# emmyoh/zebra

Measured on AMD Instinct MI355X. Metric: queries/sec, higher is better.
Workload: dtype f32

## Files before the change

### include/zebra_hip.h

```cpp
#ifndef ZEBRA_HIP_H
#define ZEBRA_HIP_H

#include <stddef.h>
#include <stdint.h>

#ifdef __cplusplus
extern "C" {
#endif

#if defined(__GNUC__)
#define ZH_API __attribute__((visibility("default")))
#else
#define ZH_API
#endif

typedef struct zh_index zh_index;

typedef enum zh_status {
    ZH_OK = 0,
    ZH_EINVAL = -1,
    ZH_ENOMEM = -2,
    ZH_EHIP = -3,
    ZH_ESTATE = -4,
    ZH_ELIMIT = -5,
// ... 169 lines not shown
ZH_API int zh_distance_batch(int metric, int cosine_mode, const float *a, const float *q, size_t n, size_t dim,
                      uint64_t *out_keys, int device);
ZH_API int zh_distance_pair(int metric, int cosine_mode, const float *a, const float *b, size_t dim, uint64_t *out_key,
                     int device);

ZH_API int zh_merge_topk_device(int device, uint32_t n_shards, size_t b, size_t k, const uint64_t *d_ids,
                         const uint64_t *d_keys, const uint32_t *d_counts, uint64_t *d_out_ids,
                         uint64_t *d_out_keys, uint32_t *d_out_counts, void *stream);

ZH_API size_t zh_packed_result_words(size_t b, size_t k);
ZH_API int zh_merge_topk_packed_device(int device, uint32_t n_shards, size_t b, size_t k, const uint64_t *d_packed,
                                uint64_t *d_out_ids, uint64_t *d_out_keys, uint32_t *d_out_counts, void *stream);

typedef struct zh_shard_group zh_shard_group;
#define ZH_UNIQUE_ID_BYTES 128
ZH_API int zh_shard_unique_id(uint8_t out_id[ZH_UNIQUE_ID_BYTES]);
ZH_API int zh_shard_group_create(zh_index *shard, const uint8_t id[ZH_UNIQUE_ID_BYTES], uint32_t n_ranks, uint32_t rank,
                                 zh_shard_group **out);
ZH_API void zh_shard_group_destroy(zh_shard_group *grp);
ZH_API uint32_t zh_shard_group_ranks(const zh_shard_group *grp);
ZH_API uint32_t zh_shard_group_rank(const zh_shard_group *grp);
ZH_API int zh_shard_search_batch_device(zh_shard_group *grp, const float *d_q, size_t b, size_t k, int metric, int cosine_mode,
                                        uint64_t *d_out_ids, uint64_t *d_out_keys, uint32_t *d_out_counts);
ZH_API int zh_shard_search_batch(zh_shard_group *grp, const float *q, size_t b, size_t k, int metric, int cosine_mode,
                                 uint64_t *out_ids, uint64_t *out_keys, uint32_t *out_counts);
typedef struct zh_shard_ctx zh_shard_ctx;
ZH_API int zh_shard_ctx_create(zh_shard_group *grp, zh_shard_ctx **out);
ZH_API void zh_shard_ctx_destroy(zh_shard_ctx *ctx);
ZH_API int zh_shard_search_begin(zh_shard_ctx *ctx, const float *d_q, size_t b, size_t k, int metric, int cosine_mode);
ZH_API int zh_shard_search_finish(zh_shard_ctx *ctx, uint64_t *d_out_ids, uint64_t *d_out_keys, uint32_t *d_out_counts);
ZH_API int zh_shard_search_wait(zh_shard_ctx *ctx);
ZH_API int zh_shard_search_begin_window(zh_shard_ctx *ctx, const float *const *d_q, size_t n_batches, size_t b, size_t k,
                                        int metric, int cosine_mode);
ZH_API int zh_shard_search_finish_window(zh_shard_ctx *ctx, uint64_t *const *d_out_ids, uint64_t *const *d_out_keys,
                                         uint32_t *const *d_out_counts);
ZH_API void *zh_shard_ctx_stream(const zh_shard_ctx *ctx);
ZH_API const uint64_t *zh_shard_ctx_local_result(const zh_shard_ctx *ctx);
ZH_API size_t zh_shard_exchange_words(size_t b, size_t k);
ZH_API uint64_t zh_shard_status_word(int status, uint32_t visits_per_query);
ZH_API int zh_shard_verdict(const uint64_t *status_words, uint32_t n_ranks, uint32_t rank, uint32_t *out_first_failed_rank,
                            uint32_t *out_max_visits_per_query, int *out_all_elimit);

ZH_API int zh_synth_queries_device(int device, float *d_out, uint64_t seed_rows, uint64_t seed_q, uint64_t n_rows,
                            uint64_t b0, size_t b, uint32_t dim, int kind, void *stream);

typedef struct zh_ref_forest zh_ref_forest;
ZH_API int zh_ref_forest_decode(uint32_t dim, size_t n_trees, const uint8_t *const *values, const size_t *lens,
                                size_t n_vectors, const uint8_t *uuids, zh_ref_forest **out, uint64_t *out_unknown_ids);
ZH_API int zh_ref_forest_view(const zh_ref_forest *forest, zh_forest_view *out);
ZH_API void zh_ref_forest_free(zh_ref_forest *forest);
ZH_API int zh_ref_tree_encode(const zh_forest_view *forest, uint32_t dim, uint32_t tree, const uint8_t *uuids,
                              uint64_t n_rows, uint8_t *out, size_t cap, size_t *out_len);

typedef struct zh_ref_header {
    uint8_t uuid[16];
    uint64_t max_node_size;
    uint64_t num_trees;
    int32_t metric;
    int32_t power;
    uint64_t model_off, model_len;
} zh_ref_header;
ZH_API int zh_ref_header_decode(const uint8_t *bytes, size_t len, int metric, size_t model_len, zh_ref_header *out);
ZH_API int zh_ref_header_encode(const zh_ref_header *header, const uint8_t *model_bytes, uint8_t *out, size_t cap, size_t *out_len);

typedef struct zh_debug_pair {
    uint32_t row;
    uint32_t query;
    uint32_t lo, hi;
    float raw_s, raw_a2;
    uint32_t flags;
    uint32_t visit;
} zh_debug_pair;
typedef struct zh_debug_scan_info {
    uint32_t approx_scan;
    uint32_t queries, top_k;
    int32_t metric, cosine_mode;
    uint32_t raw_kept;
    uint32_t overflow;
    float bound_const;
    float row_rho, rho_norm;
    uint64_t pairs, visits;
} zh_debug_scan_info;
ZH_API int zh_debug_keep_raw(zh_index *idx, int on);
ZH_API int zh_debug_scan_pairs(zh_index *idx, zh_search_ctx *ctx, zh_debug_scan_info *info, zh_debug_pair *out, size_t cap, float *qmeta);

ZH_API int zh_set_profiling(zh_index *idx, int level);
ZH_API int zh_stats(zh_index *idx, zh_stats_t *out);
ZH_API int zh_stats_reset(zh_index *idx);
ZH_API int zh_set_dense_levels(zh_index *idx, int levels);
ZH_API int zh_set_sweep_mode(zh_index *idx, int mode);
ZH_API int zh_set_hash_mode(zh_index *idx, int mode);

ZH_API const char *zh_last_error(void);
ZH_API const char *zh_version(void);
ZH_API int zh_trim_device_memory(void);

#ifdef __cplusplus
}
#endif
#endif
```

### zebra_amd/_ffi.py

```python
import ctypes as C
import os

_HERE = os.path.dirname(os.path.abspath(__file__))
LIB_PATH = os.path.join(_HERE, "lib", "libzebra_hip.so")

ZH_OK = 0
ZH_EINVAL, ZH_ENOMEM, ZH_EHIP, ZH_ESTATE, ZH_ELIMIT, ZH_EUNSUPPORTED, ZH_EPEER = -1, -2, -3, -4, -5, -6, -7
COSINE, L2SQ, L2 = 0, 1, 2
CHEBYSHEV, CANBERRA, BRAY_CURTIS, MANHATTAN, L3, L4, HAMMING, MINKOWSKI, PNORM = 3, 4, 5, 6, 7, 8, 9, 10, 11
COSINE_PARITY, COSINE_CORRECTED = 0, 1
MAX_TOPK = 1024


class ZhError(RuntimeError):
    def __init__(self, code, msg):
        super().__init__(f"zebra_hip error {code}: {msg}")
        self.code = code


class Options(C.Structure):
    _fields_ = [("dim", C.c_uint32), ("max_node_size", C.c_uint32), ("num_trees", C.c_uint32),
                ("seed", C.c_uint64), ("device", C.c_int32), ("id_base", C.c_uint64),
                ("reserve_rows", C.c_uint64)]

# ... 58 lines not shown


class CompactInfo(C.Structure):
    _fields_ = [("rows_before", C.c_uint64), ("rows_after", C.c_uint64), ("rows_moved", C.c_uint64), ("bytes_moved", C.c_uint64),
                ("scratch_bytes", C.c_uint64), ("capacity_rows", C.c_uint64), ("copy_bytes_released", C.c_uint64), ("ms", C.c_double)]

    def as_dict(self):
        return {k: getattr(self, k) for k, _ in self._fields_}


COMPACT_BOUNCE_BYTES = 256 << 20

_vp, _u64, _u32, _sz, _i = C.c_void_p, C.c_uint64, C.c_uint32, C.c_size_t, C.c_int
SYMBOLS = [
    ("zh_options_default", None, [_vp]),
    ("zh_index_create", _i, [_vp, _vp]),
    ("zh_index_destroy", None, [_vp]),
    ("zh_index_clear", _i, [_vp]),
    ("zh_index_add", _i, [_vp, _vp, _sz, _vp]),
    ("zh_index_append", _i, [_vp, _vp, _sz, _vp]),
    ("zh_index_append_device", _i, [_vp, _vp, _sz]),
    ("zh_index_append_synthetic", _i, [_vp, _sz, _u64, _u64, _i]),
    ("zh_index_build", _i, [_vp]),
    ("zh_index_remove", _i, [_vp, _vp, _sz, _vp, _vp]),
    ("zh_index_deduplicate", _i, [_vp, _vp, _sz, _vp]),
    ("zh_index_compact", _i, [_vp, _vp, _sz, _vp]),
    ("zh_index_set_forest", _i, [_vp, _vp]),
    ("zh_index_forest_sizes", _i, [_vp, _vp]),
    ("zh_index_get_forest", _i, [_vp] * 8),
    ("zh_index_count", _u64, [_vp]),
    ("zh_index_num_trees", _u32, [_vp]),
    ("zh_index_stored_rows", _u64, [_vp]),
    ("zh_index_dim", _u32, [_vp]),
    ("zh_index_device", C.c_int32, [_vp]),
    ("zh_index_id_base", _u64, [_vp]),
    ("zh_index_rows_device", _vp, [_vp]),
    ("zh_index_sweep_stream", _vp, [_vp]),
    ("zh_index_read_rows", _i, [_vp, _u64, _sz, _vp]),
    ("zh_hash_signs", _i, [_vp, _vp, _sz, _vp, _vp]),
    ("zh_search_batch", _i, [_vp, _vp, _sz, _sz, _i, _i, _vp, _vp, _vp]),
    ("zh_search_batch_device", _i, [_vp, _vp, _sz, _sz, _i, _i, _vp, _vp, _vp, _vp]),
    ("zh_search_exact_batch", _i, [_vp, _vp, _sz, _sz, _i, _i, _vp, _vp, _vp]),
    ("zh_search_exact_batch_device", _i, [_vp, _vp, _sz, _sz, _i, _i, _vp, _vp, _vp, _vp]),
    ("zh_search_exact_info", _i, [_vp, _vp]),
    ("zh_search_ctx_create", _i, [_vp, _vp]),
    ("zh_search_ctx_destroy", None, [_vp]),
    ("zh_search_begin", _i, [_vp, _vp, _sz, _sz, _i, _i, _vp]),
    ("zh_search_finish", _i, [_vp, _vp, _vp, _vp, _vp]),
    ("zh_search_wait", _i, [_vp]),
    ("zh_search_begin_window", _i, [_vp, _vp, _sz, _sz, _sz, _i, _i, _vp]),
    ("zh_search_finish_window", _i, [_vp, _vp, _vp, _vp, _vp]),
    ("zh_distance_batch", _i, [_i, _i, _vp, _vp, _sz, _sz, _vp, _i]),
    ("zh_distance_pair", _i, [_i, _i, _vp, _vp, _sz, _vp, _i]),
    ("zh_merge_topk_device", _i, [_i, _u32, _sz, _sz, _vp, _vp, _vp, _vp, _vp, _vp, _vp]),
    ("zh_packed_result_words", _sz, [_sz, _sz]),
    ("zh_merge_topk_packed_device", _i, [_i, _u32, _sz, _sz, _vp, _vp, _vp, _vp, _vp]),
    ("zh_shard_unique_id", _i, [_vp]),
    ("zh_shard_group_create", _i, [_vp, _vp, _u32, _u32, _vp]),
    ("zh_shard_group_destroy", None, [_vp]),
    ("zh_shard_group_ranks", _u32, [_vp]),
    ("zh_shard_group_rank", _u32, [_vp]),
    ("zh_shard_search_batch_device", _i, [_vp, _vp, _sz, _sz, _i, _i, _vp, _vp, _vp]),
    ("zh_shard_search_batch", _i, [_vp, _vp, _sz, _sz, _i, _i, _vp, _vp, _vp]),
    ("zh_shard_ctx_create", _i, [_vp, _vp]),
    ("zh_shard_ctx_destroy", None, [_vp]),
    ("zh_shard_search_begin", _i, [_vp, _vp, _sz, _sz, _i, _i]),
    ("zh_shard_search_finish", _i, [_vp, _vp, _vp, _vp]),
    ("zh_shard_search_wait", _i, [_vp]),
    ("zh_shard_search_begin_window", _i, [_vp, _vp, _sz, _sz, _sz, _i, _i]),
    ("zh_shard_search_finish_window", _i, [_vp, _vp, _vp, _vp]),
    ("zh_shard_ctx_stream", _vp, [_vp]),
    ("zh_shard_ctx_local_result", _vp, [_vp]),
    ("zh_shard_exchange_words", _sz, [_sz, _sz]),
    ("zh_shard_status_word", _u64, [_i, _u32]),
    ("zh_shard_verdict", _i, [_vp, _u32, _u32, _vp, _vp, _vp]),
    ("zh_synth_queries_device", _i, [_i, _vp, _u64, _u64, _u64, _u64, _sz, _u32, _i, _vp]),
    ("zh_ref_forest_decode", _i, [_u32, _sz, _vp, _vp, _sz, _vp, _vp, _vp]),
    ("zh_ref_forest_view", _i, [_vp, _vp]),
    ("zh_ref_forest_free", None, [_vp]),
    ("zh_ref_tree_encode", _i, [_vp, _u32, _u32, _vp, _u64, _vp, _sz, _vp]),
    ("zh_ref_header_decode", _i, [_vp, _sz, _i, _sz, _vp]),
    ("zh_ref_header_encode", _i, [_vp, _vp, _vp, _sz, _vp]),
    ("zh_debug_keep_raw", _i, [_vp, _i]),
    ("zh_debug_scan_pairs", _i, [_vp, _vp, _vp, _vp, _sz, _vp]),
    ("zh_set_profiling", _i, [_vp, _i]),
    ("zh_stats", _i, [_vp, _vp]),
    ("zh_stats_reset", _i, [_vp]),
    ("zh_set_dense_levels", _i, [_vp, _i]),
    ("zh_set_sweep_mode", _i, [_vp, _i]),
    ("zh_set_hash_mode", _i, [_vp, _i]),
    ("zh_last_error", C.c_char_p, []),
    ("zh_version", C.c_char_p, []),
    ("zh_trim_device_memory", _i, []),
]

_lib = None


def lib():
    global _lib
    if _lib is None:
        if not os.path.exists(LIB_PATH):
            raise ImportError(f"{LIB_PATH} is missing: build it with `python -c 'import __graft_entry__ as g; "
                              f"g.build()'` or `make -C zebra_amd/csrc` (there is no CPU fallback)")
        L = C.CDLL(LIB_PATH)
        for name, res, args in SYMBOLS:
            fn = getattr(L, name)
            fn.restype = res
            fn.argtypes = args
        _lib = L
    return _lib


def check(rc):
    if rc != ZH_OK:
        raise ZhError(rc, lib().zh_last_error().decode("utf-8", "replace"))
```

### zebra_amd/csrc/zh_api.hip

```cpp
#include <algorithm>
#include <atomic>
#include <chrono>
#include <condition_variable>
#include <cmath>
#include <deque>
#include <cstdarg>
#include <cstdio>
#include <cstring>
#include <mutex>
#include <shared_mutex>
#include <new>
#include <string>
#include <thread>
#include <vector>

#include "zh_internal.h"

static thread_local std::string g_err;

static int fail(int code, const char *fmt, ...) {
    char buf[512];
    va_list ap;
    va_start(ap, fmt);
    vsnprintf(buf, sizeof buf, fmt, ap);
// ... 12 lines not shown
int zh_set_error(int code, const char *fmt, ...) {
    char buf[512];
    va_list ap;
    va_start(ap, fmt);
    vsnprintf(buf, sizeof buf, fmt, ap);
    va_end(ap);
    g_err = buf;
    return code;
}

extern "C" const char *zh_last_error(void) { return g_err.c_str(); }
extern "C" const char *zh_version(void) { return "zebra-hip 0.1 (gfx950)"; }

struct DevBuf {
    void *p = nullptr;
    size_t cap = 0;
    bool defer = false;
    std::vector<void *> old;
    size_t old_bytes = 0;
    int ensure(size_t bytes, bool keep = false, hipStream_t s = nullptr) {
        if (bytes <= cap) return ZH_OK;
        if (defer) bytes += bytes / 8;
        if (defer && old_bytes + cap > (size_t(2) << 30)) {
            for (void *o : old) hipFree(o);
            old.clear();
            old_bytes = 0;
        }
        size_t ncap = std::max(bytes, cap + cap / 2);
        ncap = (ncap + 255) & ~size_t(255);
        void *np = nullptr;
        hipError_t e = hipMalloc(&np, ncap);
        if (e != hipSuccess) {
            ncap = (bytes + 255) & ~size_t(255);
            e = hipMalloc(&np, ncap);
        }
        if (e != hipSuccess) return fail(ZH_ENOMEM, "hipMalloc(%zu bytes): %s", ncap, hipGetErrorString(e));
        if (keep && p && cap) {
            e = hipMemcpyAsync(np, p, cap, hipMemcpyDeviceToDevice, s);
            if (e == hipSuccess) e = hipStreamSynchronize(s);
            if (e != hipSuccess) { hipFree(np); return fail(ZH_EHIP, "grow copy: %s", hipGetErrorString(e)); }
        }
        if (p) { if (defer) { old.push_back(p); old_bytes += cap; } else hipFree(p); }
        p = np;
        cap = ncap;
        return ZH_OK;
    }
    void release() {
        if (p) hipFree(p);
        for (void *o : old) hipFree(o);
        old.clear();
        old_bytes = 0;
        p = nullptr;
        cap = 0;
    }
    template <typename T>
    T *as() const { return reinterpret_cast<T *>(p); }
};

struct zh_search_ctx {
    zh_index *ix = nullptr;
    DevBuf wQQ, wBits, wCounts, wInline, wRowBase, wCandBase, wVisitBase, wTotals, wVisits, wKeys, wCandKeys, wCandIds,
        wLeafCount, wLeafFill, wGroupBase, wGroupRowBase, wGroups, wGroupRowOff, wWaveGroup, wVisitBits, wNodeVisit, wScore, wJunkBits, wZeros, wQnorm, wQpad, wFixList, wLogPool, wLogHead, wLogCtl,
        wPfRows, wPfCounts, wPfKeys, wPfIds, wPfAmb, wPfCtl, wUnc, wQh, wQmeta, wApList, wApCount, wApEx, wApExKeys, wApCtl, wRaw;
    ZhApprox dbg_ap{};
    bool dbg_valid = false, dbg_raw = false;
    size_t log_chunks = 0;
    ZhTotals *h_totals = nullptr;
    hipEvent_t ev[6] = {};
    hipEvent_t ev_totals = nullptr, ev_emit = nullptr, ev_sw0 = nullptr, ev_sw1 = nullptr;
    bool ev_ok = false;
    int state = 0;
    bool trivial = false;
    const float *dQ = nullptr;
    size_t B = 0, k = 0;
    size_t nwin = 1, bwin = 0;
    DevBuf wQwin, wOutWin;
    int metric = 0, mode = 0;
    uint32_t P_dense = 0, wpq = 0;
    hipStream_t s = nullptr;
    ZhTotals tot{};
    bool scan = false;
    bool approx_f32rows = false;
    bool approx_fused = false;
    bool approx_bytes = false;
    bool approx = false, approx_mfma = false, approx_leaf = false;
    uint32_t *h_ap = nullptr;
    bool score_hash = false;
    uint32_t score_Bp = 0;
    bool lazy_fix = false;
    bool prefilter = false, prefilter_off_once = false, stream_ordered = false;
    uint32_t pf_cap = 0;
    uint32_t *h_pf = nullptr;
    std::vector<const float *> sv_q;
    std::vector<uint64_t *> sv_ids, sv_keys;
    std::vector<uint32_t *> sv_counts;
    hipStream_t sv_heavy = nullptr;
    std::vector<DevBuf *> all_bufs() {
        return {&wQQ, &wBits, &wCounts, &wInline, &wRowBase, &wCandBase, &wVisitBase, &wTotals, &wVisits, &wKeys,
                &wCandKeys, &wCandIds, &wLeafCount, &wLeafFill, &wGroupBase, &wGroupRowBase, &wGroups, &wGroupRowOff, &wWaveGroup, &wVisitBits, &wNodeVisit, &wScore, &wJunkBits, &wZeros, &wQnorm, &wQpad, &wFixList,
                &wLogPool, &wLogHead, &wLogCtl, &wQwin, &wOutWin, &wPfRows, &wPfCounts, &wPfKeys, &wPfIds, &wPfAmb, &wPfCtl, &wUnc,
                &wQh, &wQmeta, &wApList, &wApCount, &wApEx, &wApExKeys, &wApCtl, &wRaw};
    }
    void release_all() {
        for (DevBuf *b : all_bufs()) b->release();
        if (ev_ok) { for (auto &e : ev) hipEventDestroy(e); hipEventDestroy(ev_totals); hipEventDestroy(ev_emit); hipEventDestroy(ev_sw0); hipEventDestroy(ev_sw1); ev_ok = false; }
        if (h_totals) { hipHostFree(h_totals); h_totals = nullptr; }
        if (h_pf) { hipHostFree(h_pf); h_pf = nullptr; }
        if (h_ap) { hipHostFree(h_ap); h_ap = nullptr; }
    }
};

struct zh_index {
    zh_options opt{};
    int device = 0;
    hipStream_t stream = nullptr;
    hipStream_t sweep_stream = nullptr;
    std::shared_mutex mu;

    DevBuf X;
    uint64_t n_rows = 0;

    DevBuf node_plane, node_left, node_right, node_pack, roots, planes, consts, leaf_ids;
    uint32_t n_nodes = 0, n_planes = 0, n_trees = 0;
    uint64_t n_leaf_ids = 0;
    std::vector<int32_t> h_plane, h_left, h_right;
    std::vector<uint32_t> h_roots;
    std::vector<uint32_t> planes_below_level;
    std::vector<uint32_t> h_leaf_ids;
    std::vector<uint8_t> h_dead;
    uint64_t n_dead = 0;
    std::vector<uint32_t> h_live;
    uint64_t h_live_rows = ~0ull;
    uint64_t h_live_dead = ~0ull;
    uint64_t h_live_gen = ~0ull;
    uint64_t rows_gen = 1, dead_gen = 1;
    uint32_t max_leaf_len = 0;
    DevBuf blk_recs, blk_upper, blk_roots;
    uint32_t n_blocks = 0, n_upper = 0;
    bool blocks_valid = false;
    bool blocks_inner = false;
    size_t blk_recs_b = 0;
    std::mutex blk_mu;
    DevBuf row_leaf;
    bool row_leaf_valid = false, row_leaf_failed = false;
    std::atomic<uint32_t> batches_since_change{0};
    DevBuf row_half, row_meta, row_rho_dev;
    std::atomic<bool> row_half_failed{false};
    DevBuf row_half128;
    std::atomic<uint64_t> h128_rows{0}, h128_gen{0};
    int h128_ex = 0;
    float h128_rho = 0.f;
    std::atomic<bool> h128_failed{false};
    bool h128_bytes = false, h128_not_bytes = false;
    std::atomic<uint64_t> scale_rows{0}, scale_gen{0};
    float row_rho = 0.f;
    DevBuf scan_perm, row_leaf_p;
    bool row_order_off = false;
    uint32_t order_keys = 0;
    double order_worth = 0;
    uint64_t perm_rows = 0, row_leaf_gen = 0, row_leaf_p_gen = 0, perm_gen = 0, row_leaf_p_perm = 0;
    uint64_t row_leaf_rows = 0;

    zh_search_ctx dctx;
    DevBuf wQ, wOutIds, wOutKeys, wOutCounts;
    DevBuf ex_live, ex_bits, ex_QQ, ex_keys, ex_visits, ex_cbase, ex_ckeys, ex_cids, ex_run_ids, ex_run_keys, ex_run_counts, ex_Q, ex_ids, ex_kout, ex_counts,
        ex_Qh, ex_qmeta, ex_tau, ex_cnt, ex_lid, ex_llo, ex_lhi, ex_scr, ex_over;
    uint64_t ex_live_rows = ~0ull, ex_live_gen = ~0ull, ex_n_live = 0;
    zh_exact_info ex_info{};

    bool broken = false;
    bool rows_torn = false;
    int dense_levels = -1;
    bool debug_keep_raw = false;
    std::atomic<int> sweep_mode{0};
    std::atomic<uint32_t> approx_strikes{0};
    std::atomic<bool> mfma_f32_off{false};
    std::atomic<bool> fused_off{false};
    int hash_mode = 0;
    DevBuf plane_samples;
    bool samples_valid = false;
    DevBuf row_hn2, row_norm;
    uint64_t norm_rows = 0, norm_gen = 0;
    DevBuf plane_hab;
    uint32_t hab_planes = 0;
    uint64_t hab_rows = 0, hab_gen = 0;
    DevBuf leaf_meta;
    bool leaf_meta_valid = false;
    uint64_t meta_rows = 0, meta_gen = 0;
    std::atomic<uint32_t> prefilter_strikes{0};
    bool scan_unsafe = false;
    double visits_per_pair = 0;
    int profiling = 0;
    std::mutex stats_mu;
    zh_stats_t stats{};
    struct CombineReq {
        const float *q; size_t b, k; int metric, mode;
        uint64_t *ids, *keys; uint32_t *counts;
        int rc = 0; std::string err;
        std::mutex m; std::condition_variable cv; bool done = false, lead = false;
    };
    struct Lane {
        zh_search_ctx ctx;
        bool init = false, busy = false;
        hipStream_t s = nullptr;
        zh_search_ctx ctx2;
        bool init2 = false;
        hipStream_t s2 = nullptr;
        zh_search_ctx ctx3;
        bool init3 = false;
        hipStream_t s3 = nullptr;
        zh_search_ctx ctx4;
        bool init4 = false;
        hipStream_t s4 = nullptr;
        hipEvent_t ev_d2h[4] = {nullptr, nullptr, nullptr, nullptr};
        DevBuf wQ, wOutIds, wOutKeys, wOutCounts;
        void *h_stage = nullptr;
        size_t h_stage_cap = 0;
    };
    std::mutex cmu;
    std::deque<CombineReq *> cpend;
    bool cleader = false;
    size_t clast = 0;
    Lane lanes[1];
};

static const char *const k_torn_msg = "an earlier zh_index_compact failed after rows had begun to move: the stored rows are inconsistent; "
                                      "zh_index_clear the index and store them again";
static int set_device(const zh_index *ix) {
    hipError_t e = hipSetDevice(ix->device);
    if (e != hipSuccess) return fail(ZH_EHIP, "hipSetDevice(%d): %s", ix->device, hipGetErrorString(e));
    return ZH_OK;
}

static ZhForestDev forest_dev(const zh_index *ix) {
    ZhForestDev f;
    f.node_plane = ix->node_plane.as<int32_t>();
    f.node_left = ix->node_left.as<int32_t>();
    f.node_right = ix->node_right.as<int32_t>();
    f.node_pack = ix->node_pack.as<int4>();
    f.roots = ix->roots.as<uint32_t>();
    f.planes = ix->planes.as<float>();
    f.consts = ix->consts.as<float>();
    f.leaf_ids = ix->leaf_ids.as<uint32_t>();
    f.n_nodes = ix->n_nodes;
    f.n_planes = ix->n_planes;
    f.n_trees = ix->n_trees;
    f.group = zh_group_size(ix->opt.dim);
    return f;
}

static int ctx_init(zh_search_ctx *c, zh_index *ix) {
    c->ix = ix;
    for (DevBuf *b : c->all_bufs()) b->defer = true;
    hipError_t e = hipHostMalloc((void **)&c->h_totals, sizeof(ZhTotals), hipHostMallocDefault);
    if (e != hipSuccess) return fail(ZH_ENOMEM, "hipHostMalloc: %s", hipGetErrorString(e));
    e = hipHostMalloc((void **)&c->h_pf, 4 * sizeof(uint32_t), hipHostMallocDefault);
// ... 1836 lines not shown
                                   c->wCandBase.as<uint64_t>(), c->wVisitBase.as<uint64_t>(), c->wVisits.as<ZhVisit>(),
                                   c->wLeafCount.as<uint32_t>(), c->wLeafFill.as<uint32_t>(), c->wGroupBase.as<uint32_t>(),
                                   c->wGroupRowBase.as<uint64_t>(), c->wGroups.as<ZhGroup>(), c->wGroupRowOff.as<uint64_t>(), s));
        const uint64_t pairs = (uint64_t)B * T;
        const uint64_t want = tot.visits / (ZH_LOG_CHUNK - 1) + std::min<uint64_t>(pairs, tot.visits / (ZH_INLINE_VISITS + 1)) + 16;
        static const bool fixed = getenv("ZH_WALK_LOG_FIXED") != nullptr;
        if (!fixed && want > c->log_chunks) {
            const size_t chunks = (size_t)(want + want / 2);
            if (c->wLogPool.ensure(chunks * ZH_LOG_CHUNK * sizeof(uint2)) == ZH_OK) c->log_chunks = chunks;
        }
    }
    c->scan = choose_scan(ix, tot, c->metric, B, k);
    if (c->scan && (!ix->row_leaf_valid || ix->row_leaf_rows != ix->n_rows)) {
        std::lock_guard<std::mutex> lk(ix->blk_mu);
        if ((!ix->row_leaf_valid || ix->row_leaf_rows != ix->n_rows) && !ix->row_leaf_failed && (rc = build_row_leaf(ix))) return rc;
        if (!ix->row_leaf_valid || ix->row_leaf_rows != ix->n_rows) c->scan = false;
    }
    if (c->scan) {
        const size_t nn = std::max<uint32_t>(ix->n_nodes, 1);
        if ((rc = c->wVisitBits.ensure((nn + 31) / 32 * 4))) return rc;
        if ((rc = c->wNodeVisit.ensure(nn * sizeof(uint4)))) return rc;
        HIPCHK(zh_launch_node_visits(c->wLeafCount.as<uint32_t>(), c->wGroupBase.as<uint32_t>(), c->wGroups.as<ZhGroup>(), ix->n_nodes,
                                     c->wVisitBits.as<uint32_t>(), c->wNodeVisit.as<uint4>(), s));
    }
    if (!c->scan)
        HIPCHK(zh_launch_wave_groups(c->wGroups.as<ZhGroup>(), c->wGroupRowOff.as<uint64_t>(), tot.groups, c->wWaveGroup.as<uint32_t>(), s));
    c->approx = c->scan && use_approx(ix, tot, B, k, c->metric);
    c->approx_leaf = false; c->approx_bytes = false;
    if (!c->scan && use_approx_leaf(ix, tot, B, k, c->metric)) {
        bool ok = false;
        const char *be = getenv("ZH_S128H_BYTES"), *ke = getenv("ZH_S128H_KERNEL"), *de = getenv("ZH_S128H_DMA");
        const bool want_bytes = !(be && be[0] == '0') && !(ke && ke[0] == 'r') && !(de && de[0] == '1');
        std::lock_guard<std::mutex> lk(ix->blk_mu);
        if ((rc = ensure_row_half128(ix, &ok, want_bytes))) return rc;
        c->approx = c->approx_leaf = ok;
        c->approx_bytes = ok && ix->h128_bytes;
    }
    ZhApprox ap{};
    bool mfma = c->approx && !c->approx_leaf && mfma_wanted(ix) && B < (1u << 23) - 1;
    const uint2 *scan_row_leaf = ix->row_leaf.as<uint2>();
    if (mfma) {
        std::lock_guard<std::mutex> lk(ix->blk_mu);
        if ((rc = ensure_row_half(ix, &mfma))) return rc;
        if (mfma && ix->perm_rows) {
            if ((rc = ensure_row_leaf_p(ix))) return rc;
            if (!ix->perm_rows) {
                ix->row_order_off = true;
                ix->scale_gen = 0;
                if ((rc = ensure_row_half(ix, &mfma))) return rc;
            } else
                scan_row_leaf = ix->row_leaf_p.as<uint2>();
        }
    }
    c->approx_mfma = mfma;
    c->approx_f32rows = mfma && ix->row_half.p == nullptr;
    if (c->approx) {
        const char *cap_e = getenv("ZH_APX_CAPS");
        unsigned e_capq = 0, e_excap = 0, e_exrows = 0;
        if (cap_e) sscanf(cap_e, "%u,%u,%u", &e_capq, &e_excap, &e_exrows);
        const uint32_t capq = e_capq ? std::min(e_capq, 8192u) : (ix->approx_strikes.load() ? 8192u : 4096u);
        const uint32_t ex_cap = e_excap ? e_excap : (uint32_t)std::min<uint64_t>(std::max<uint64_t>(4096, tot.visits / 4 + 1024), 1u << 24);
        const uint32_t ex_rows = e_exrows ? e_exrows : (uint32_t)std::min<uint64_t>(std::max<uint64_t>(1u << 20, tot.rows / 16), 1u << 26);
        if ((rc = c->wQh.ensure(B * d * 2)) || (rc = c->wQmeta.ensure(B * sizeof(float4))) || (rc = c->wApList.ensure((size_t)B * capq * 12)) ||
            (rc = c->wApCount.ensure(B * 8 + std::max<uint64_t>(tot.visits, 1) * 4)) || (rc = c->wApEx.ensure((size_t)ex_cap * 8)) || (rc = c->wApExKeys.ensure((size_t)ex_rows * 20)) ||
            (rc = c->wApCtl.ensure(ZH_APX_CTL_WORDS * 4)))
            return rc;
        ap.Qh = c->wQh.p; ap.qmeta = c->wQmeta.as<float4>(); ap.iv = c->wKeys.as<uint64_t>();
        ap.list_lo = c->wApList.as<uint32_t>(); ap.list_hi = ap.list_lo + (size_t)B * capq; ap.list_id = ap.list_hi + (size_t)B * capq;
        ap.qcount = c->wApCount.as<uint32_t>(); ap.capq = capq; ap.qtau = ap.qcount + B; ap.tauv = ap.qtau + B;
        ap.ex_visits = c->wApEx.as<uint2>(); ap.ex_cap = ex_cap;
        ap.ex_keys = c->wApExKeys.as<uint64_t>(); ap.ex_ckeys = ap.ex_keys + ex_rows; ap.ex_cids = reinterpret_cast<uint32_t *>(ap.ex_ckeys + ex_rows);
        ap.ex_rows_cap = ex_rows; ap.ctl = c->wApCtl.as<uint32_t>();
        ap.n_queries = (uint32_t)B; ap.iv_cap = tot.rows;
        ap.mfma = mfma ? 1u : 0u; ap.row_half = mfma ? ix->row_half.p : nullptr; ap.row_meta = mfma ? ix->row_meta.as<float2>() : nullptr;
        ap.row_rho = mfma ? ix->row_rho : 0.f;
        if (c->approx_leaf) { ap.mfma = 2u; ap.row_rho = ap.rho_norm = c->approx_bytes ? 0.f : ix->h128_rho; }
        const char *pte = getenv("ZH_S128H_PRETEST");
        ap.nx_max = c->approx_leaf && c->approx_bytes && !(pte && pte[0] == '0') ? 2885.1f : 0.f;
        HIPCHK(hipMemsetAsync(c->wApCount.p, 0, B * 4, s));
        HIPCHK(hipMemsetAsync(ap.qtau, 0xFF, B * 4, s));
        HIPCHK(hipMemsetAsync(c->wApCtl.p, 0, ZH_APX_CTL_WORDS * 4, s));
        HIPCHK(zh_launch_qhalf(c->dQ, (uint32_t)B, d, c->wQh.p, c->wQmeta.as<float4>(), c->approx_leaf ? 2 : (mfma ? 1 : 0), s));
    }
    HIPCHK(hipEventRecord(c->ev[2], s));
    hipStream_t hs = heavy ? heavy : s;
    if (hs != s) { HIPCHK(hipEventRecord(c->ev_emit, s)); HIPCHK(hipStreamWaitEvent(hs, c->ev_emit, 0)); }
    HIPCHK(hipEventRecord(c->ev_sw0, hs));
    c->approx_fused = false;
    if (c->approx_leaf && k <= 64 && !ix->debug_keep_raw) {
        const char *fe = getenv("ZH_S128H_FUSED"), *ke = getenv("ZH_S128H_KERNEL"), *de = getenv("ZH_S128H_DMA");
        const bool lean = !(ke && ke[0] == 'r') && !(de && de[0] == '1');
        c->approx_fused = lean && (fe ? fe[0] == '1' : (!ix->fused_off && tot.rows >= 1024 * std::max<uint64_t>(tot.visits, 1)));
    }
    const int kinda = c->metric != ZH_COSINE ? 0 : (c->mode == ZH_COSINE_PARITY ? 2 : 1);
    if (c->approx_leaf)
        HIPCHK(zh_launch_sweep128h(ix->row_half128.p, c->wQh.p, ldexpf(1.f, ix->h128_ex - 14), c->wGroups.as<ZhGroup>(), c->wGroupRowOff.as<uint64_t>(),
                                   tot.groups, c->wWaveGroup.as<uint32_t>(), f.leaf_ids, tot.group_rows, c->wKeys.as<uint64_t>(), hs,
                                   c->approx_fused ? &ap : nullptr, kinda, (uint32_t)k, zh_approx_bound(c->metric, d, 2), c->approx_bytes));
    else if (c->approx)
        HIPCHK(zh_launch_scan_approx(ix->X.as<float>(), d, ix->n_rows, ap, mfma ? scan_row_leaf : ix->row_leaf.as<uint2>(), T, c->wVisitBits.as<uint32_t>(),
                                     c->wNodeVisit.as<uint4>(), c->wGroups.as<ZhGroup>(), f.group, c->metric, c->mode, hs));
    else if (c->scan)
        HIPCHK(zh_launch_scan_sweep(ix->X.as<float>(), d, ix->n_rows, c->dQ, c->wQQ.as<float>(), ix->row_leaf.as<uint2>(), T,
                                    c->wVisitBits.as<uint32_t>(), c->wNodeVisit.as<uint4>(), c->wGroups.as<ZhGroup>(), f.group,
                                    c->metric, c->mode, c->wKeys.as<uint64_t>(), nullptr, hs));
    else
        HIPCHK(zh_launch_sweep(ix->X.as<float>(), d, c->dQ, c->wQQ.as<float>(), c->wGroups.as<ZhGroup>(),
                               c->wGroupRowOff.as<uint64_t>(), tot.groups, c->wWaveGroup.as<uint32_t>(), f.leaf_ids,
                               tot.group_rows, c->metric, c->mode, c->wKeys.as<uint64_t>(), hs));
    HIPCHK(hipEventRecord(c->ev_sw1, hs));
    if (hs != s) HIPCHK(hipStreamWaitEvent(s, c->ev_sw1, 0));
    HIPCHK(hipEventRecord(c->ev[3], s));
    const uint32_t *run_if = nullptr;
    c->dbg_valid = c->approx;
    c->dbg_raw = false;
    if (c->approx) {
        c->dbg_ap = ap;
        if (ix->debug_keep_raw && tot.rows) {
            if ((rc = c->wRaw.ensure(tot.rows * 8))) return rc;
            HIPCHK(hipMemcpyAsync(c->wRaw.p, c->wKeys.p, tot.rows * 8, hipMemcpyDeviceToDevice, s));
            c->dbg_raw = true;
        }
        if (c->approx_fused) HIPCHK(zh_launch_exact_register(c->wVisits.as<ZhVisit>(), tot.visits, (uint32_t)k, ap, s));
        else HIPCHK(zh_launch_select_interval(c->wVisits.as<ZhVisit>(), tot.visits, (uint32_t)k, f.leaf_ids, ap, c->metric, c->mode, d, s));
        HIPCHK(hipEventRecord(c->ev[4], s));
        HIPCHK(zh_launch_final_interval(c->wVisits.as<ZhVisit>(), ix->X.as<float>(), d, c->dQ, c->wQQ.as<float>(), (uint32_t)B, (uint32_t)k,
                                        f.leaf_ids, c->metric, c->mode, ix->opt.id_base, ap, dOutIds, dOutKeys, dOutCounts, ix->max_leaf_len, s));
        HIPCHK(hipMemcpyAsync(c->h_ap, c->wApCtl.p, ZH_APX_CTL_WORDS * 4, hipMemcpyDeviceToHost, s));
        run_if = ap.ctl + 1;
        if (c->approx_leaf)
            HIPCHK(zh_launch_sweep(ix->X.as<float>(), d, c->dQ, c->wQQ.as<float>(), c->wGroups.as<ZhGroup>(), c->wGroupRowOff.as<uint64_t>(), tot.groups,
                                   c->wWaveGroup.as<uint32_t>(), f.leaf_ids, tot.group_rows, c->metric, c->mode, c->wKeys.as<uint64_t>(), s, run_if));
        else
            HIPCHK(zh_launch_scan_sweep(ix->X.as<float>(), d, ix->n_rows, c->dQ, c->wQQ.as<float>(), ix->row_leaf.as<uint2>(), T,
                                        c->wVisitBits.as<uint32_t>(), c->wNodeVisit.as<uint4>(), c->wGroups.as<ZhGroup>(), f.group,
                                        c->metric, c->mode, c->wKeys.as<uint64_t>(), run_if, s));
    }
    HIPCHK(zh_launch_select(c->wVisits.as<ZhVisit>(), tot.visits, f.leaf_ids, c->wKeys.as<uint64_t>(),
                            c->wCandKeys.as<uint64_t>(), c->wCandIds.as<uint32_t>(), ix->max_leaf_len, run_if, s));
    if (!c->approx) HIPCHK(hipEventRecord(c->ev[4], s));
    HIPCHK(zh_launch_final(c->wCandBase.as<uint64_t>(), (uint32_t)B, T, (uint32_t)k, c->wCandKeys.as<uint64_t>(),
                           c->wCandIds.as<uint32_t>(), ix->opt.id_base, dOutIds, dOutKeys, dOutCounts, run_if, s));
    for (size_t j = 0; j < nwin && nwin > 1; j++) {
        HIPCHK(hipMemcpyAsync(outIds[j], dOutIds + j * bwin * k, bwin * k * 8, hipMemcpyDeviceToDevice, s));
        HIPCHK(hipMemcpyAsync(outKeys[j], dOutKeys + j * bwin * k, bwin * k * 8, hipMemcpyDeviceToDevice, s));
        HIPCHK(hipMemcpyAsync(outCounts[j], dOutCounts + j * bwin, bwin * 4, hipMemcpyDeviceToDevice, s));
    }
    HIPCHK(hipEventRecord(c->ev[5], s));
    c->state = 2;
    return ZH_OK;
}

int ctx_wait(zh_search_ctx *c) {
    zh_index *ix = c->ix;
    if (c->state == 1) return fail(ZH_ESTATE, "zh_search_wait: the batch was begun but not finished");
    if (c->state != 2) return ZH_OK;
    c->state = 0;
    HIPCHK(hipEventSynchronize(c->ev[5]));
    if (c->trivial) return ZH_OK;
    const bool pf = c->prefilter;
    const uint32_t pf_amb = pf ? c->h_pf[0] : 0, pf_flags = pf ? c->h_pf[1] : 0, pf_exact = pf ? c->h_pf[2] : 0;
    if (pf_flags) {
        {
            std::lock_guard<std::mutex> lk(ix->stats_mu);
            ix->stats.prefilter_fallbacks_accum++;
            ix->stats.prefilter_last_overflow = pf_flags;
        }
        ix->prefilter_strikes.fetch_add(1);
        const std::vector<const float *> q = c->sv_q;
        const std::vector<uint64_t *> ids = c->sv_ids, keys = c->sv_keys;
        const std::vector<uint32_t *> counts = c->sv_counts;
        c->prefilter_off_once = true;
        int rc = ctx_begin(c, q.data(), c->nwin, c->bwin, c->k, c->metric, c->mode, c->s);
        if (!rc) rc = ctx_finish(c, ids.data(), keys.data(), counts.data(), c->sv_heavy);
        c->prefilter_off_once = false;
        if (rc) return rc;
        return ctx_wait(c);
    }
    if (pf) ix->prefilter_strikes = 0;
    const ZhTotals tot = c->tot;
    uint64_t uniq = 0;
    if (ix->profiling >= 2 && tot.visits && !pf) {
        std::vector<ZhVisit> hv(tot.visits);
        HIPCHK(hipMemcpy(hv.data(), c->wVisits.p, tot.visits * sizeof(ZhVisit), hipMemcpyDeviceToHost));
// ... 110 lines not shown

extern "C" int zh_search_ctx_create(zh_index *ix, zh_search_ctx **out) {
    if (!ix || !out) return fail(ZH_EINVAL, "zh_search_ctx_create: null argument");
    int rc = set_device(ix);
    if (rc) return rc;
    zh_search_ctx *c = new (std::nothrow) zh_search_ctx();
    if (!c) return fail(ZH_ENOMEM, "out of host memory");
    if ((rc = ctx_init(c, ix))) { c->release_all(); delete c; return rc; }
    *out = c;
    return ZH_OK;
}
extern "C" void zh_search_ctx_destroy(zh_search_ctx *c) {
    if (!c) return;
    hipSetDevice(c->ix->device);
    if (c->state == 2) hipEventSynchronize(c->ev[5]);
    else if (c->state == 1 && c->s) hipStreamSynchronize(c->s);
    c->release_all();
    delete c;
}
extern "C" int zh_search_begin(zh_search_ctx *c, const float *d_q, size_t b, size_t k, int metric, int mode, void *stream) {
    if (!c || (b && !d_q)) return fail(ZH_EINVAL, "zh_search_begin: null argument");
    if (k > ZH_MAX_TOPK) return fail(ZH_ELIMIT, "top_k %zu > ZH_MAX_TOPK (%u)", k, ZH_MAX_TOPK);
    int rc = check_metric(metric, mode);
    if (rc) return rc;
    if ((rc = set_device(c->ix))) return rc;
    return ctx_begin(c, &d_q, 1, b, k, metric, mode, stream ? (hipStream_t)stream : c->ix->stream);
}
extern "C" int zh_search_begin_window(zh_search_ctx *c, const float *const *d_q, size_t n_batches, size_t b, size_t k, int metric,
                                      int mode, void *stream) {
    if (!c || !d_q || n_batches == 0 || n_batches > ZH_MAX_WINDOW) return fail(ZH_EINVAL, "zh_search_begin_window: bad argument (1..%u batches)", ZH_MAX_WINDOW);
    for (size_t j = 0; j < n_batches; j++)
        if (b && !d_q[j]) return fail(ZH_EINVAL, "zh_search_begin_window: null query pointer");
    if (k > ZH_MAX_TOPK) return fail(ZH_ELIMIT, "top_k %zu > ZH_MAX_TOPK (%u)", k, ZH_MAX_TOPK);
    int rc = check_metric(metric, mode);
    if (rc) return rc;
    if ((rc = set_device(c->ix))) return rc;
    return ctx_begin(c, d_q, n_batches, b, k, metric, mode, stream ? (hipStream_t)stream : c->ix->stream);
}
extern "C" int zh_search_finish(zh_search_ctx *c, uint64_t *d_out_ids, uint64_t *d_out_keys, uint32_t *d_out_counts,
                                void *sweep_stream) {
    if (!c) return fail(ZH_EINVAL, "zh_search_finish: null context");
    if (c->B && (!d_out_counts || (c->k && (!d_out_ids || !d_out_keys)))) return fail(ZH_EINVAL, "zh_search_finish: null output");
    if (c->nwin != 1) return fail(ZH_ESTATE, "zh_search_finish: the context holds a window; use zh_search_finish_window");
    int rc = set_device(c->ix);
    if (rc) return rc;
    return ctx_finish(c, &d_out_ids, &d_out_keys, &d_out_counts, (hipStream_t)sweep_stream);
}
extern "C" int zh_search_finish_window(zh_search_ctx *c, uint64_t *const *d_out_ids, uint64_t *const *d_out_keys,
                                       uint32_t *const *d_out_counts, void *sweep_stream) {
    if (!c || !d_out_ids || !d_out_keys || !d_out_counts) return fail(ZH_EINVAL, "zh_search_finish_window: null argument");
    for (size_t j = 0; j < c->nwin && c->bwin; j++)
        if (!d_out_counts[j] || (c->k && (!d_out_ids[j] || !d_out_keys[j]))) return fail(ZH_EINVAL, "zh_search_finish_window: null output");
    int rc = set_device(c->ix);
    if (rc) return rc;
    return ctx_finish(c, d_out_ids, d_out_keys, d_out_counts, (hipStream_t)sweep_stream);
}
double zh_index_visits_per_pair(zh_index *ix) {
    std::lock_guard<std::mutex> lk(ix->stats_mu);
    return ix->visits_per_pair;
}
void zh_search_ctx_stream_ordered(zh_search_ctx *c) {
    if (c) c->stream_ordered = true;
}
void zh_search_ctx_abandon(zh_search_ctx *c) {
    if (c && c->state == 1) c->state = 0;
}
extern "C" int zh_search_wait(zh_search_ctx *c) {
    if (!c) return fail(ZH_EINVAL, "zh_search_wait: null context");
    int rc = set_device(c->ix);
    if (rc) return rc;
    return ctx_wait(c);
}

extern "C" int zh_trim_device_memory(void) {
    return ZH_OK;
}

extern "C" int zh_debug_keep_raw(zh_index *ix, int on) {
    if (!ix) return fail(ZH_EINVAL, "zh_debug_keep_raw: null index");
    std::unique_lock<std::shared_mutex> lk(ix->mu);
    ix->debug_keep_raw = on != 0;
    return ZH_OK;
}
extern "C" int zh_debug_scan_pairs(zh_index *ix, zh_search_ctx *ctx, zh_debug_scan_info *info, zh_debug_pair *out, size_t cap, float *qmeta) {
    if (!ix || !info || (cap && !out)) return fail(ZH_EINVAL, "zh_debug_scan_pairs: null argument");
    std::unique_lock<std::shared_mutex> lk(ix->mu, std::defer_lock);
    if (!ctx) lk.lock();
    zh_search_ctx *c = ctx ? ctx : &ix->dctx;
    if (c->ix != ix) return fail(ZH_EINVAL, "zh_debug_scan_pairs: the context belongs to another index");
    if (c->state != 0) return fail(ZH_ESTATE, "zh_debug_scan_pairs: the context has a batch in flight");
    int rc = set_device(ix);
    if (rc) return rc;
    memset(info, 0, sizeof(*info));
    if (!c->dbg_valid) return ZH_OK;
    if (c->approx_leaf && c->approx_fused)
        return fail(ZH_ESTATE, "zh_debug_scan_pairs: the batch's sweep was fused (no per-pair results exist); call zh_debug_keep_raw(idx, 1) first");
    const ZhTotals tot = c->tot;
    const ZhApprox &ap = c->dbg_ap;
    info->approx_scan = c->approx_leaf ? 3 : (c->approx_mfma ? 2 : 1);
    info->queries = (uint32_t)c->B; info->top_k = (uint32_t)c->k; info->metric = c->metric; info->cosine_mode = c->mode;
    info->raw_kept = c->dbg_raw ? 1 : 0; info->overflow = c->h_ap[1];
    info->bound_const = zh_approx_bound(c->metric, ix->opt.dim, (int)ap.mfma);
    info->row_rho = ap.row_rho; info->rho_norm = ap.rho_norm;
    info->pairs = tot.rows; info->visits = tot.visits;
    HIPCHK(hipDeviceSynchronize());
    if (qmeta) HIPCHK(hipMemcpy(qmeta, ap.qmeta, c->B * sizeof(float4), hipMemcpyDeviceToHost));
    if (!cap) return ZH_OK;
    if (cap < tot.rows) return fail(ZH_ELIMIT, "zh_debug_scan_pairs: %llu pairs, room for %zu", (unsigned long long)tot.rows, cap);
    std::vector<ZhVisit> hv(tot.visits);
    std::vector<uint64_t> iv(tot.rows), raw(c->dbg_raw ? tot.rows : 0);
    std::vector<uint32_t> lids(ix->n_leaf_ids);
    if (tot.visits) HIPCHK(hipMemcpy(hv.data(), c->wVisits.p, tot.visits * sizeof(ZhVisit), hipMemcpyDeviceToHost));
    if (tot.rows) HIPCHK(hipMemcpy(iv.data(), c->wKeys.p, tot.rows * 8, hipMemcpyDeviceToHost));
    if (c->dbg_raw && tot.rows) HIPCHK(hipMemcpy(raw.data(), c->wRaw.p, tot.rows * 8, hipMemcpyDeviceToHost));
    if (ix->n_leaf_ids) HIPCHK(hipMemcpy(lids.data(), ix->leaf_ids.p, ix->n_leaf_ids * 4, hipMemcpyDeviceToHost));
    for (size_t i = 0; i < tot.rows; i++) { out[i].row = out[i].query = 0xFFFFFFFFu; out[i].flags = 0; out[i].visit = 0xFFFFFFFFu; }
    for (size_t v = 0; v < hv.size(); v++) {
        const ZhVisit &z = hv[v];
        if (z.row_off + z.len > tot.rows || (uint64_t)z.leaf_off + z.len > ix->n_leaf_ids) return fail(ZH_ESTATE, "zh_debug_scan_pairs: visit %zu out of range", v);
        const uint32_t fl = (z.take ? 1u : 0u) | ((z.take && z.take < z.len && z.take < c->k) ? 2u : 0u);
        for (uint32_t i = 0; i < z.len; i++) {
            zh_debug_pair &o = out[z.row_off + i];
            o.row = lids[(size_t)z.leaf_off + i]; o.query = z.b; o.visit = (uint32_t)v; o.flags = fl;
            const uint64_t w = iv[z.row_off + i];
            o.lo = (uint32_t)w; o.hi = (uint32_t)(w >> 32);
            o.raw_s = o.raw_a2 = 0.f;
            if (c->dbg_raw) { const uint64_t r = raw[z.row_off + i]; uint32_t a = (uint32_t)r, b2 = (uint32_t)(r >> 32); memcpy(&o.raw_s, &a, 4); memcpy(&o.raw_a2, &b2, 4); }
        }
    }
    return ZH_OK;
}

static size_t host_window_queries(const zh_index *ix, bool wander) {
    const char *e = getenv("ZH_HOST_WINDOW");
    const size_t forced = e ? (size_t)atoll(e) : (size_t)0;
    if (forced) return forced;
    const uint32_t d = ix->opt.dim;
    if (wander) {
        const size_t w = ((size_t)1 << 28) / std::max<uint64_t>(ix->n_rows, 1) / 64 * 64;
        return std::min<size_t>(std::max<size_t>(w, 64), 1024);
    }
    return d >= 512 ? 2048 : (d >= 256 ? 1024 : 4096);
}
static size_t host_windows_wanted(zh_index *ix, size_t B, size_t k, bool *wander) {
    const bool off = getenv("ZH_NO_HOST_WINDOWS") != nullptr;
    if (off || ix->n_trees == 0 || ix->n_rows == 0) return 0;
    double vpp;
    {
        std::lock_guard<std::mutex> lk(ix->stats_mu);
        vpp = ix->visits_per_pair;
    }
    if (!(vpp > 0)) {
        if ((size_t)ix->opt.max_node_size >= 2 * k + 2) return 0;
        vpp = 1000.0;
    }
    const size_t wq = host_window_queries(ix, vpp > 4.0);
    if (B < 2 * wq && B < wq + wq / 2) return 0;
    *wander = vpp > 4.0;
    return wq;
}
#ifndef ZH_HOST_AHEAD_WANDER
#define ZH_HOST_AHEAD_WANDER 2
#endif
static int search_host_windows(zh_index *ix, zh_index::Lane &ln, size_t wq, int ahead, const float *q, size_t B, size_t k, int metric, int mode, uint64_t *out_ids,
                               uint64_t *out_keys, uint32_t *out_counts) {
    const uint32_t d = ix->opt.dim;
    int rc;
    auto init_ctx = [&](zh_search_ctx *c, hipStream_t *st, bool *flag) -> int {
        if (*flag) return ZH_OK;
        int r = ctx_init(c, ix);
        if (r) { c->release_all(); return r; }
        int lo = 0, hi = 0;
        hipDeviceGetStreamPriorityRange(&lo, &hi);
        hipError_t e = hipStreamCreateWithPriority(st, hipStreamNonBlocking, hi);
        for (auto &ev : ln.ev_d2h)
            if (e == hipSuccess && !ev) e = hipEventCreateWithFlags(&ev, hipEventDisableTiming);
        if (e != hipSuccess) {
            c->release_all();
            if (*st) { hipStreamDestroy(*st); *st = nullptr; }
            return fail(ZH_EHIP, "host windows: %s", hipGetErrorString(e));
        }
        *flag = true;
        return ZH_OK;
    };
    if ((rc = init_ctx(&ln.ctx2, &ln.s2, &ln.init2))) return rc;
    if (ahead >= 1 && init_ctx(&ln.ctx3, &ln.s3, &ln.init3) != ZH_OK) ahead = 0;
    if (ahead >= 2 && init_ctx(&ln.ctx4, &ln.s4, &ln.init4) != ZH_OK) ahead = 1;
    const int NC = 2 + ahead;
    const size_t A = (size_t)ahead;
    const size_t nw = (B + wq - 1) / wq, per = (B + nw - 1) / nw;
    const size_t off_ids = B * d * 4, off_keys = off_ids + B * k * 8, off_counts = off_keys + B * k * 8, need = off_counts + B * 4;
    if (need > ln.h_stage_cap) {
        if (ln.h_stage) hipHostFree(ln.h_stage);
        ln.h_stage = nullptr; ln.h_stage_cap = 0;
        const size_t cap = need + need / 2;
        hipError_t e = hipHostMalloc(&ln.h_stage, cap, hipHostMallocDefault);
        if (e != hipSuccess) return fail(ZH_ENOMEM, "hipHostMalloc(%zu): %s", cap, hipGetErrorString(e));
        ln.h_stage_cap = cap;
    }
    uint8_t *hs = static_cast<uint8_t *>(ln.h_stage);
    float *dQ = ln.wQ.as<float>();
    uint64_t *dIds = ln.wOutIds.as<uint64_t>(), *dKeys = ln.wOutKeys.as<uint64_t>();
    uint32_t *dCounts = ln.wOutCounts.as<uint32_t>();
    uint64_t *hIds = reinterpret_cast<uint64_t *>(hs + off_ids), *hKeys = reinterpret_cast<uint64_t *>(hs + off_keys);
    uint32_t *hCounts = reinterpret_cast<uint32_t *>(hs + off_counts);
    zh_search_ctx *ctxs[4] = {&ln.ctx, &ln.ctx2, &ln.ctx3, &ln.ctx4};
    hipStream_t str[4] = {ln.s, ln.s2, ln.s3, ln.s4};
    auto win = [&](size_t w, size_t *b0, size_t *nb) { *b0 = w * per; *nb = std::min(per, B - *b0); };
// ... 601 lines not shown
```

### zebra_amd/csrc/zh_approx.hip

```cpp

#include <cstdlib>

#include "zh_internal.h"
#include "zh_device.h"

typedef _Float16 f16x8 __attribute__((ext_vector_type(8)));

#ifndef ZH_APX_G768
#define ZH_APX_G768 2
#endif
#ifndef ZH_APX_G128
#define ZH_APX_G128 8
#endif
uint32_t zh_approx_groups(uint32_t d) {
    switch (d) {
    case 128: return ZH_APX_G128;
    case 256: case 384: return 4;
    case 768: return ZH_APX_G768;
    case 512: case 1024: return 2;
    default: return 0;
    }
}
bool zh_approx_pays(uint32_t d) { return d >= 384; }

float zh_approx_bound(int metric, uint32_t d, int mfma) {
    const double u = 5.9604644775390625e-8, c0 = (d + 255) / 256 + 8.0, ops = mfma ? 33.0 * (d / 128) + 2.0 + (mfma == 2 ? 40.0 : 0.0) : 0.0;
    if (metric == ZH_COSINE) return (float)(1.01 * (2.0 * c0 + 80.0 + 2.0 * ops) * u);
    return (float)(1.01 * (c0 + 100.0 + ops) * u);
}

__device__ __forceinline__ _Float16 f16_no_subnormal(float v) {
    const _Float16 h = (_Float16)v;
    return fabsf((float)h) < 6.103515625e-05f ? (_Float16)0.f : h;
}

template <int G>
__global__ __launch_bounds__(64) void qhalf_kernel(const float *__restrict__ Q, uint32_t B, uint32_t d, _Float16 *__restrict__ Qh,
                                                    float4 *__restrict__ qmeta) {
    constexpr uint32_t LG = 64 / G;
    const uint32_t b = blockIdx.x, lane = threadIdx.x;
    const float *q = Q + (size_t)b * d;
    float m = 0.f, s2 = 0.f;
    bool bad = false;
    for (uint32_t e = lane; e < d; e += 64) {
        const float v = q[e];
        bad |= !(v - v == 0.f);
        m = fmaxf(m, fabsf(v));
        s2 = __builtin_fmaf(v, v, s2);
    }
    m = wave_butterfly<OpMax>(m);
    s2 = wave_sum_canonical(s2);
    bad = __ballot(bad) != 0;
    float sigma = 1.f, inv = 1.f;
    if (!bad && m > 0.f) {
        int ex = 0;
        (void)frexpf(m, &ex);
        if (ex < -90 || ex > 90) bad = true;
        else { sigma = ldexpf(1.f, 14 - ex); inv = ldexpf(1.f, ex - 14); }
    }
    float d2 = 0.f;
    for (uint32_t e = lane; e < d; e += 64) {
        const float v = bad ? 0.f : q[e];
        const _Float16 h = f16_no_subnormal(v * sigma);
        const float df = v - (float)h * inv;
        d2 = __builtin_fmaf(df, df, d2);
        const uint32_t j = e / (4 * LG), rem = e % (4 * LG), l = rem / 4, t = rem % 4, i = j / 2, wh = j % 2;
        Qh[(size_t)b * d + ((size_t)(i * LG + l)) * 8 + wh * 4 + t] = h;
    }
    d2 = wave_sum_canonical(d2);
    if (lane == 0) {
        float4 o;
        if (bad || !(s2 - s2 == 0.f)) o = make_float4(NAN, NAN, NAN, NAN);
        else o = make_float4(inv, s2, sqrtf(s2) * (1.0f + 1e-5f), sqrtf(d2) * 1.001f);
        qmeta[b] = o;
    }
}

hipError_t zh_launch_qhalf(const float *dQ, uint32_t B, uint32_t d, void *dQh, float4 *dQmeta, int layout, hipStream_t s) {
    if (!B) return hipSuccess;
    const uint32_t G = layout == 2 ? 64 : (layout == 1 ? 16 : zh_approx_groups(d));
    if (G == 64) hipLaunchKernelGGL(qhalf_kernel<64>, dim3(B), dim3(64), 0, s, dQ, B, d, (_Float16 *)dQh, dQmeta);
    else if (G == 16) hipLaunchKernelGGL(qhalf_kernel<16>, dim3(B), dim3(64), 0, s, dQ, B, d, (_Float16 *)dQh, dQmeta);
    else if (G == 8) hipLaunchKernelGGL(qhalf_kernel<8>, dim3(B), dim3(64), 0, s, dQ, B, d, (_Float16 *)dQh, dQmeta);
// ... 272 lines not shown
        const uint64_t row = row0 + i;
        const float *x = X + (size_t)(perm && row < perm_rows ? perm[row] : row) * d;
        float m = 0.f, a2 = 0.f;
        bool bad = false;
        for (uint32_t e = lane; e < d; e += 64) {
            const float v = x[e];
            bad |= !(v - v == 0.f);
            m = fmaxf(m, fabsf(v));
            a2 = __builtin_fmaf(v, v, a2);
        }
        m = wave_butterfly<OpMax>(m);
        a2 = wave_sum_canonical(a2);
        bad = __ballot(bad) != 0;
        bool usable = false;
        float sigma = 1.f, inv = __uint_as_float(0x7FC00000u);
        if (!bad) {
            int ex = 14;
            if (m > 0.f) (void)frexpf(m, &ex);
            if (ex >= -100 && ex <= 100) { usable = true; sigma = ldexpf(1.f, 14 - ex); inv = ldexpf(1.f, ex - 14); }
        }
        float s2 = 0.f, d2 = 0.f;
        _Float16 *tile = Xh + ((size_t)(row >> 4) * NS * 64 + (row & 15)) * 8;
        for (uint32_t e = lane; e < d; e += 64) {
            const float v = x[e] * sigma;
            const _Float16 hv = usable ? f16_no_subnormal(v) : (_Float16)0.f;
            const float df = v - (float)hv;
            s2 = __builtin_fmaf(v, v, s2);
            d2 = __builtin_fmaf(df, df, d2);
            const uint32_t st = e >> 5, w = e & 31, hh = (w & 15) >> 2, j = (w & 3) + ((w >> 4) << 2);
            if (Xh) tile[((size_t)st * 64 + hh * 16) * 8 + j] = hv;
        }
        s2 = wave_sum_canonical(s2);
        d2 = wave_sum_canonical(d2);
        if (usable && s2 > 0.f) rho_w = fmaxf(rho_w, sqrtf(d2) * 1.001f / (sqrtf(s2) * 0.9999f));
        if (lane == 0) rowMeta[row] = make_float2(a2, inv);
    }
    if (lane == 0 && rho_w > 0.f) atomicMax(rhoMax, __float_as_uint(rho_w));
}

hipError_t zh_launch_row_half(const float *dX, uint64_t row0, uint64_t n_rows, uint32_t d, void *dXh, float2 *dRowMeta, uint32_t *dRhoMax,
                              const uint32_t *dPerm, uint64_t perm_rows, hipStream_t s) {
    if (!n_rows) return hipSuccess;
    const uint64_t blocks = std::min<uint64_t>((n_rows + 3) / 4, 256 * 32);
    hipLaunchKernelGGL(row_half_kernel, dim3((uint32_t)blocks), dim3(256), 0, s, dX, row0, n_rows, d, (_Float16 *)dXh, dRowMeta, dRhoMax, dPerm, perm_rows);
    return hipGetLastError();
}

__global__ __launch_bounds__(256) void permute_row_leaf_kernel(const uint2 *__restrict__ rowLeaf, const uint32_t *__restrict__ perm, uint64_t perm_rows,
                                                               uint64_t n_entries, uint32_t T, uint2 *__restrict__ out) {
    for (uint64_t e = (uint64_t)blockIdx.x * blockDim.x + threadIdx.x; e < n_entries; e += (uint64_t)gridDim.x * blockDim.x) {
        const uint64_t p = e / T, t = e % T;
        out[e] = rowLeaf[(size_t)(p < perm_rows ? perm[p] : p) * T + t];
    }
}
hipError_t zh_launch_permute_row_leaf(const uint2 *dRowLeaf, const uint32_t *dPerm, uint64_t perm_rows, uint64_t n_rows, uint32_t T, uint2 *dOut, hipStream_t s) {
    const uint64_t n = n_rows * T;
    if (!n) return hipSuccess;
    hipLaunchKernelGGL(permute_row_leaf_kernel, dim3((uint32_t)std::min<uint64_t>((n + 255) / 256, 256 * 64)), dim3(256), 0, s, dRowLeaf, dPerm, perm_rows, n, T, dOut);
    return hipGetLastError();
}

#ifndef ZH_MFMA_CL
#define ZH_MFMA_CL 0
#endif
#ifdef ZH_SCAN_GUARD
#define ZH_GUARD(cond, bit) ((cond) ? true : (atomicOr(guard, (bit)), false))
#else
#define ZH_GUARD(cond, bit) true
#endif
#ifdef ZH_SCAN_PROF
__device__ unsigned long long zh_scan_prof_buf[16];
extern "C" __attribute__((visibility("default"))) int zh_debug_scan_prof(uint64_t *out, uint32_t words, int reset) {
    static const unsigned long long zero[16] = {};
    if (reset) return (int)hipMemcpyToSymbol(HIP_SYMBOL(zh_scan_prof_buf), zero, sizeof(zero));
    return (int)hipMemcpyFromSymbol(out, HIP_SYMBOL(zh_scan_prof_buf), (size_t)words * 8);
}
#define SP(...) __VA_ARGS__
#else
#define SP(...)
#endif
#ifndef ZH_MFMA_WAVES
#define ZH_MFMA_WAVES 3
#endif
template <int D, bool F32ROWS>
__global__ __launch_bounds__(256) __attribute__((amdgpu_waves_per_eu(D > 768 ? 2 : ZH_MFMA_WAVES, D > 768 ? 2 : ZH_MFMA_WAVES)))
void scan_mfma_kernel(const u32x4v *__restrict__ Xh, const float *__restrict__ Xf, const float2 *__restrict__ rowMeta,
                                                         const uint4 *__restrict__ Qh, const uint2 *__restrict__ rowLeaf, uint32_t T,
                                                         uint32_t RW, const uint32_t *__restrict__ visitBits,
                                                         const uint4 *__restrict__ nodeVisit, const ZhGroup *__restrict__ groups,
                                                         uint32_t GRP, uint64_t row_begin, uint64_t row_end, uint64_t *__restrict__ iv,
                                                         uint32_t *__restrict__ colStats ,
                                                         uint32_t nq, uint64_t iv_cap, uint32_t *__restrict__ guard) {
    constexpr int NS = D / 32;
    constexpr int NL = D / 64;
    constexpr int CL = ZH_MFMA_CL ? ZH_MFMA_CL : (NL % 4 == 0 ? 2 : 3);
    constexpr int NCH = NL / CL;
    static_assert(D % 128 == 0 && NL % CL == 0 && NCH % 2 == 0, "four accumulators; the chunk registers alternate with a static parity");
    __shared__ uint64_t pair_list[4][ZH_APX_CAP > CL * 256 ? ZH_APX_CAP : CL * 256];
    __shared__ uint64_t tile_list[4][ZH_APX_CAP];
    __shared__ uint32_t col_query[4][ZH_APX_CAP];
    __shared__ uint32_t tile_start[4][36];
    __shared__ f32x4v acc_lds[4][64];
    __shared__ float2 row_meta[4][16];
    const uint32_t lane = threadIdx.x & 63, c16 = lane & 15, h = lane >> 4;
    const uint32_t wid = (uint32_t)__builtin_amdgcn_readfirstlane((int)(threadIdx.x >> 6));
    const uint64_t wave = (uint64_t)blockIdx.x * (blockDim.x >> 6) + wid;
    const uint64_t r0 = row_begin + wave * RW;
    if (r0 >= row_end) return;
    SP(const uint64_t sp0 = clock64();)
    const uint32_t nr = (uint32_t)(row_end - r0 < RW ? row_end - r0 : RW);
    const uint32_t n_ent = nr * T;
    const uint2 *__restrict__ ent = rowLeaf + (size_t)r0 * T;
    uint32_t eGb[ZH_SCAN_NE], eWithin[ZH_SCAN_NE], eC[ZH_SCAN_NE], off[ZH_SCAN_NE], eB0[ZH_SCAN_NE];
    uint64_t eK0[ZH_SCAN_NE];
    const uint32_t P = scan_phase1(lane, n_ent, ent, visitBits, nodeVisit, eGb, eWithin, eC, off, eB0, eK0);
    if (P == 0) return;
    SP(const uint64_t sp1 = clock64();)
    uint64_t *list = pair_list[wid];
    const bool listed = P <= ZH_APX_CAP;
    auto pack = [](uint32_t rl, uint32_t b, uint64_t slot) { return slot | ((uint64_t)b << 36) | ((uint64_t)rl << 60); };
#pragma unroll
    for (int j = 0; j < ZH_SCAN_NE; j++) {
        const uint32_t e = lane + 64u * j, c = eC[j];
        if (c && listed && ZH_GUARD(off[j] + c <= (uint32_t)ZH_APX_CAP && e / T < 16u, 32u)) {
            const uint32_t rl = e / T, gb = eGb[j];
            list[off[j]] = pack(rl, eB0[j], eK0[j] + eWithin[j]);
            for (uint32_t sidx = 1; sidx < c; sidx++) {
                const ZhGroup *gp = groups + gb + sidx / GRP;
                list[off[j] + sidx] = pack(rl, gp->b[sidx % GRP], gp->key_off[sidx % GRP] + eWithin[j]);
            }
        }
    }
    SP(__builtin_amdgcn_s_waitcnt(0); const uint64_t sp2 = clock64();)
    f16x8 A[NS];
    if constexpr (!F32ROWS) {
        const u32x4v *tp = Xh + (size_t)(r0 >> 4) * (NS * 64) + lane;
#pragma unroll
        for (int st = 0; st < NS; st++) A[st] = __builtin_bit_cast(f16x8, __builtin_nontemporal_load(tp + 64 * st));
        if (lane < 16) row_meta[wid][lane] = rowMeta[r0 + (lane < nr ? lane : 0u)];
        __builtin_amdgcn_fence(__ATOMIC_RELEASE, "wavefront");
        __builtin_amdgcn_wave_barrier();
    } else {
        if (lane < 16) row_meta[wid][lane] = rowMeta[r0 + (lane < nr ? lane : 0u)];
        __builtin_amdgcn_fence(__ATOMIC_RELEASE, "wavefront");
        __builtin_amdgcn_wave_barrier();
        const float inv_c = row_meta[wid][c16].y;
        const bool usable_c = inv_c - inv_c == 0.f;
        const float sigma_c = usable_c ? 1.0f / inv_c : 0.f;
        f32x4v *xt = reinterpret_cast<f32x4v *>(tile_list[wid]);
        const f32x4v *X4 = reinterpret_cast<const f32x4v *>(Xf);
        const uint32_t g4 = lane >> 4, p16 = lane & 15;
        auto cvt8 = [&](const f32x4v lo, const f32x4v hi) {
            f16x8 o;
#pragma unroll
            for (int t = 0; t < 4; t++) {
                o[t] = usable_c ? f16_no_subnormal(lo[t] * sigma_c) : (_Float16)0.f;
                o[4 + t] = usable_c ? f16_no_subnormal(hi[t] * sigma_c) : (_Float16)0.f;
            }
            return o;
        };
        f32x4v Rr[4];
        auto issue_rows = [&](int kb) {
#pragma unroll
            for (int i = 0; i < 4; i++) {
                const uint32_t rr = 4u * i + g4;
                Rr[i] = __builtin_nontemporal_load(X4 + (size_t)(r0 + (rr < nr ? rr : nr - 1)) * (D / 4) + kb * 16 + p16);
            }
        };
        issue_rows(0);
#pragma unroll
        for (int kb = 0; kb < D / 64; kb++) {
#pragma unroll
            for (int i = 0; i < 4; i++) {
                const uint32_t rr = 4u * i + g4;
                xt[rr * 16 + (p16 ^ rr)] = Rr[i];
            }
            __builtin_amdgcn_fence(__ATOMIC_RELEASE, "wavefront");
            __builtin_amdgcn_wave_barrier();
            if (kb + 1 < D / 64) issue_rows(kb + 1);
#pragma unroll
            for (int s2 = 0; s2 < 2; s2++) {
                const f32x4v lo = xt[c16 * 16 + ((8u * s2 + h) ^ c16)], hi = xt[c16 * 16 + ((8u * s2 + 4u + h) ^ c16)];
                A[2 * kb + s2] = cvt8(lo, hi);
            }
            __builtin_amdgcn_fence(__ATOMIC_RELEASE, "wavefront");
            __builtin_amdgcn_wave_barrier();
        }
    }
    const float2 *rmeta = row_meta[wid];
    u32x4v *stg = reinterpret_cast<u32x4v *>(pair_list[wid]);
    const u32x4v *__restrict__ Qv = reinterpret_cast<const u32x4v *>(Qh);
    const uint32_t g8 = lane >> 3, pc = lane & 7;
    const uint32_t swA = (g8 >> 1) & 7u, swB = (4u + (g8 >> 1)) & 7u;
    const uint32_t rd0 = (c16 >> 3) * 64u + (c16 & 7u) * 8u + ((h ^ (c16 >> 1)) & 7u);
    const uint32_t rd1 = (c16 >> 3) * 64u + (c16 & 7u) * 8u + (((4u + h) ^ (c16 >> 1)) & 7u);
    auto issue = [&](uint32_t bA, uint32_t bB, int chunk, u32x4v *dst) {
        if (!ZH_GUARD(bA < nq && bB < nq, 1u)) { bA = 0; bB = 0; }
        const u32x4v *qa = Qv + (size_t)bA * (D / 8) + (size_t)(chunk * CL * 8) + (pc ^ swA);
        const u32x4v *qb = Qv + (size_t)bB * (D / 8) + (size_t)(chunk * CL * 8) + (pc ^ swB);
#pragma unroll
        for (int i = 0; i < CL; i++) { dst[2 * i] = qa[8 * i]; dst[2 * i + 1] = qb[8 * i]; }
    };
    auto to_lds = [&](const u32x4v *src) {
#pragma unroll
        for (int i = 0; i < 2 * CL; i++) stg[64 * i + lane] = src[i];
    };
    auto mfma_chunk = [&](int chunk, f32x4v *acc) {
#pragma unroll
        for (int i = 0; i < 2 * CL; i++) {
            const u32x4v v = stg[128 * (i / 2) + ((i & 1) ? rd1 : rd0)];
            const int st = chunk * 2 * CL + i;
            acc[st & 3] = __builtin_amdgcn_mfma_f32_16x16x32_f16(A[st], __builtin_bit_cast(f16x8, v), acc[st & 3], 0, 0, 0);
        }
    };
    auto emit = [&](const f32x4v *acc, uint32_t rl, uint64_t slot, bool valid) {
        const f32x4v t = (acc[0] + acc[1]) + (acc[2] + acc[3]);
        if (valid && (rl >> 2) == h) {
            const uint32_t i = rl & 3u;
            const float sv = i == 0 ? t[0] : (i == 1 ? t[1] : (i == 2 ? t[2] : t[3]));
            const float2 rm = rmeta[rl];
            if (ZH_GUARD(slot < iv_cap, 2u))
                __builtin_nontemporal_store(((uint64_t)__float_as_uint(rm.x) << 32) | __float_as_uint(sv * rm.y), iv + slot);
        }
    };
    if (listed) {
        uint32_t *tab = reinterpret_cast<uint32_t *>(tile_list[wid]);
        uint32_t *colq = col_query[wid], *tstart = tile_start[wid];
#pragma unroll
        for (int i = 0; i < 4; i++) reinterpret_cast<uint4 *>(tab)[lane + 64 * i] = make_uint4(0u, 0u, 0u, 0u);
        if (lane < 36) tstart[lane] = 0u;
        __builtin_amdgcn_fence(__ATOMIC_RELEASE, "wavefront");
        __builtin_amdgcn_wave_barrier();
        auto hash_of = [](uint32_t b) { return (b * 2654435761u) >> 22; };
        uint32_t nd = 0;
        for (uint32_t p0 = 0; p0 < P; p0 += 64) {
            const uint32_t pi = p0 + lane;
            const bool valid = pi < P;
            const uint32_t b = valid ? (uint32_t)(list[pi] >> 36) & 0xFFFFFFu : 0u, key = b + 1u;
            uint32_t hs = hash_of(b);
            bool leader = false, open = valid;
            while (__ballot(open)) {
                if (open) {
                    const uint32_t old = atomicCAS(&tab[hs], 0u, (key << 9) | 0x1FFu);
                    if (old == 0u) { leader = true; open = false; }
                    else if ((old >> 9) == key) open = false;
                    else hs = (hs + 1u) & 1023u;
                }
            }
            const unsigned long long lm = __ballot(leader);
            if (leader) {
                const uint32_t col = nd + (uint32_t)__builtin_popcountll(lm & ((1ull << lane) - 1ull));
                if (ZH_GUARD(col < (uint32_t)ZH_APX_CAP && hs < 1024u, 64u)) {
                    tab[hs] = (key << 9) | col;
                    colq[col] = b;
                }
            }
            nd += (uint32_t)__builtin_popcountll(lm);
        }
        __builtin_amdgcn_fence(__ATOMIC_RELEASE, "wavefront");
        __builtin_amdgcn_wave_barrier();
        for (uint32_t p0 = 0; p0 < P; p0 += 64) {
            const uint32_t pi = p0 + lane;
            if (pi < P) {
                const uint64_t rec = list[pi];
                const uint32_t b = (uint32_t)(rec >> 36) & 0xFFFFFFu, key = b + 1u;
                uint32_t hs = hash_of(b), w = tab[hs];
                for (uint32_t tries = 0; (w >> 9) != key && ZH_GUARD(tries < 1024u, 16u); tries++) { (void)tries; hs = (hs + 1u) & 1023u; w = tab[hs]; }
                const uint32_t col = w & 0x1FFu;
                if (!ZH_GUARD((w >> 9) == key && col < nd, 128u)) continue;
                const uint32_t pos = atomicAdd(&tstart[1 + (col >> 4)], 1u);
                list[pi] = (rec & ~(0xFFFFFFull << 36)) | ((uint64_t)(col | (pos << 9)) << 36);
            }
        }
        __builtin_amdgcn_fence(__ATOMIC_RELEASE, "wavefront");
        __builtin_amdgcn_wave_barrier();
        {
            uint32_t v = lane < 33 ? tstart[lane] : 0u;
#pragma unroll
            for (int o = 1; o < 64; o <<= 1) {
                const uint32_t u = __shfl_up(v, o);
                if (lane >= (uint32_t)o) v += u;
            }
            __builtin_amdgcn_wave_barrier();
            if (lane < 33) tstart[lane] = v;
        }
        __builtin_amdgcn_fence(__ATOMIC_RELEASE, "wavefront");
        __builtin_amdgcn_wave_barrier();
        uint64_t *tl = tile_list[wid];
        {
            uint64_t recs[ZH_APX_CAP / 64];
#pragma unroll
            for (int i = 0; i < ZH_APX_CAP / 64; i++) recs[i] = (uint32_t)(64 * i) + lane < P ? list[64 * i + lane] : ~0ull;
            __builtin_amdgcn_wave_barrier();
#pragma unroll
            for (int i = 0; i < ZH_APX_CAP / 64; i++)
                if ((uint32_t)(64 * i) + lane < P) {
                    const uint32_t cp = (uint32_t)(recs[i] >> 36) & 0xFFFFFFu, col = cp & 0x1FFu, pos = (cp >> 9) & 0x1FFu;
                    if (ZH_GUARD(tstart[col >> 4] + pos < (uint32_t)ZH_APX_CAP && col < nd, 4u | (col < nd ? 0u : 8u))) tl[tstart[col >> 4] + pos] = recs[i];
                }
        }
        __builtin_amdgcn_fence(__ATOMIC_RELEASE, "wavefront");
        __builtin_amdgcn_wave_barrier();
        const uint32_t nt = (nd + 15) / 16;
        SP(const uint64_t sp3 = clock64();)
        if (colStats && lane == 0 && (wave & 63u) == 0u) { atomicAdd(&colStats[0], nd); atomicAdd(&colStats[1], P); }
        auto col_b = [&](uint32_t t, uint32_t col) { const uint32_t ci = 16 * t + col; return colq[ci < nd ? ci : nd - 1]; };
        uint32_t bA = col_b(0, g8), bB = col_b(0, 8 + g8);
        u32x4v ra[2 * CL], rb[2 * CL];
        issue(bA, bB, 0, ra);
        SP(__builtin_amdgcn_s_waitcnt(0); const uint64_t sp4 = clock64();)
        f32x4v *al = acc_lds[wid];
        for (uint32_t t = 0; t < nt; t++) {
            f32x4v acc[4] = {{0.f, 0.f, 0.f, 0.f}, {0.f, 0.f, 0.f, 0.f}, {0.f, 0.f, 0.f, 0.f}, {0.f, 0.f, 0.f, 0.f}};
#pragma unroll
            for (int c = 0; c < NCH; c += 2) {
                issue(bA, bB, c + 1, rb);
                to_lds(ra);
                mfma_chunk(c, acc);
                if (c + 2 < NCH) issue(bA, bB, c + 2, ra);
                else {
                    bA = col_b(t + 1, g8); bB = col_b(t + 1, 8 + g8);
                    issue(bA, bB, 0, ra);
                }
                to_lds(rb);
                mfma_chunk(c + 1, acc);
            }
            al[c16 * 4 + h] = (acc[0] + acc[1]) + (acc[2] + acc[3]);
            __builtin_amdgcn_fence(__ATOMIC_RELEASE, "wavefront");
            __builtin_amdgcn_wave_barrier();
            const uint32_t pe = tstart[t + 1];
            for (uint32_t pi = tstart[t] + lane; pi < pe; pi += 64) {
                const uint64_t rec = tl[pi];
                const uint32_t rl = (uint32_t)(rec >> 60), col = (uint32_t)(rec >> 36) & 15u;
                const float sv = reinterpret_cast<const float *>(al)[col * 16 + rl];
                const float2 rm = rmeta[rl];
                if (ZH_GUARD((rec & 0xFFFFFFFFFull) < iv_cap, 2u))
                    __builtin_nontemporal_store(((uint64_t)__float_as_uint(rm.x) << 32) | __float_as_uint(sv * rm.y), iv + (rec & 0xFFFFFFFFFull));
            }
            __builtin_amdgcn_wave_barrier();
        }
        SP(if ((wave & 15u) == 0u && lane == 0) {
            __builtin_amdgcn_s_waitcnt(0);
            const uint64_t sp5 = clock64();
            atomicAdd(&zh_scan_prof_buf[0], 1ull); atomicAdd(&zh_scan_prof_buf[1], sp1 - sp0); atomicAdd(&zh_scan_prof_buf[2], sp2 - sp1);
            atomicAdd(&zh_scan_prof_buf[3], sp3 - sp2); atomicAdd(&zh_scan_prof_buf[4], sp4 - sp3); atomicAdd(&zh_scan_prof_buf[5], sp5 - sp4);
            atomicAdd(&zh_scan_prof_buf[6], (unsigned long long)nt); atomicAdd(&zh_scan_prof_buf[7], (unsigned long long)P);
            atomicAdd(&zh_scan_prof_buf[8], (unsigned long long)nd); atomicAdd(&zh_scan_prof_buf[9], sp5 - sp0);
        })
    } else {
#pragma unroll
        for (int j = 0; j < ZH_SCAN_NE; j++) {
            unsigned long long m = __ballot(eC[j] != 0);
            while (m) {
                const int ll = __builtin_ctzll(m);
                m &= m - 1;
                const uint32_t c = (uint32_t)__builtin_amdgcn_readlane((int)eC[j], ll);
                const uint32_t gb = (uint32_t)__builtin_amdgcn_readlane((int)eGb[j], ll);
                const uint32_t w = (uint32_t)__builtin_amdgcn_readlane((int)eWithin[j], ll);
                const uint32_t rl = ((uint32_t)ll + 64u * j) / T;
                for (uint32_t s0 = 0; s0 < c; s0 += 16) {
                    auto visit_b = [&](uint32_t col) { const uint32_t si = s0 + col < c ? s0 + col : c - 1; return groups[gb + si / GRP].b[si % GRP]; };
                    const uint32_t bA = visit_b(g8), bB = visit_b(8 + g8);
                    const uint32_t sidx = s0 + c16 < c ? s0 + c16 : c - 1;
                    const ZhGroup *gp = groups + gb + sidx / GRP;
                    f32x4v acc[4] = {{0.f, 0.f, 0.f, 0.f}, {0.f, 0.f, 0.f, 0.f}, {0.f, 0.f, 0.f, 0.f}, {0.f, 0.f, 0.f, 0.f}};
                    u32x4v rq[2 * CL];
#pragma unroll
                    for (int cc = 0; cc < NCH; cc++) {
                        issue(bA, bB, cc, rq);
                        to_lds(rq);
                        mfma_chunk(cc, acc);
                        __builtin_amdgcn_sched_barrier(0);
                    }
                    emit(acc, rl, gp->key_off[sidx % GRP] + w, s0 + c16 < c);
                }
            }
        }
    }
}

template <int D>
static hipError_t launch_scan_mfma_d(const float *dX, uint64_t n_rows, const ZhApprox &ap, const uint2 *dRowLeaf, uint32_t T,
                                     const uint32_t *dVisitBits, const uint4 *dNodeVisit, const ZhGroup *dGroups, uint32_t group, hipStream_t s) {
    const uint32_t RW = zh_scan_rows_per_wave(T);
    uint64_t rows_per_launch = zh_sweep_rows_per_launch(D);
    rows_per_launch = rows_per_launch / (4 * RW) * (4 * RW);
    for (uint64_t r = 0; r < n_rows; r += rows_per_launch) {
        const uint64_t r_end = r + rows_per_launch < n_rows ? r + rows_per_launch : n_rows;
        const uint64_t waves = (r_end - r + RW - 1) / RW, blocks = (waves + 3) / 4;
        if (blocks > 0x7FFFFFFFull) return hipErrorInvalidValue;
        if (ap.row_half)
            hipLaunchKernelGGL((scan_mfma_kernel<D, false>), dim3((uint32_t)blocks), dim3(256), 0, s, (const u32x4v *)ap.row_half, dX, ap.row_meta, (const uint4 *)ap.Qh, dRowLeaf, T, RW,
                               dVisitBits, dNodeVisit, dGroups, group, r, r_end, ap.iv, ap.ctl + 5, ap.n_queries, ap.iv_cap, ap.ctl + 7);
        else
            hipLaunchKernelGGL((scan_mfma_kernel<D, true>), dim3((uint32_t)blocks), dim3(256), 0, s, (const u32x4v *)nullptr, dX, ap.row_meta, (const uint4 *)ap.Qh, dRowLeaf, T, RW,
                               dVisitBits, dNodeVisit, dGroups, group, r, r_end, ap.iv, ap.ctl + 5, ap.n_queries, ap.iv_cap, ap.ctl + 7);
    }
    return hipGetLastError();
}

__global__ __launch_bounds__(256) void absmax_kernel(const float *__restrict__ X, uint64_t n, uint32_t *__restrict__ out) {
    float m = 0.f;
    for (uint64_t i = (uint64_t)blockIdx.x * blockDim.x + threadIdx.x; i < n; i += (uint64_t)gridDim.x * blockDim.x) {
        const float v = fabsf(X[i]);
        if (v - v == 0.f) m = fmaxf(m, v);
    }
    m = wave_butterfly<OpMax>(m);
    if ((threadIdx.x & 63) == 0 && m > 0.f) atomicMax(out, __float_as_uint(m));
}

__global__ __launch_bounds__(256) void row_half128_kernel(const float *__restrict__ X, uint64_t row0, uint64_t n_rows, float sigma,
                                                          _Float16 *__restrict__ Xh, uint32_t *__restrict__ rhoMax) {
    const uint32_t lane = threadIdx.x & 63;
    const uint64_t nw = (uint64_t)gridDim.x * 4;
    float rho_w = 0.f;
    for (uint64_t i = (uint64_t)blockIdx.x * 4 + (threadIdx.x >> 6); i < n_rows; i += nw) {
        const uint64_t row = row0 + i;
        const float2 x = reinterpret_cast<const float2 *>(X + (size_t)row * 128)[lane];
        const float v0 = x.x * sigma, v1 = x.y * sigma;
        bool bad = !(v0 - v0 == 0.f) || !(v1 - v1 == 0.f) || fabsf(v0) > 60000.f || fabsf(v1) > 60000.f;
        const _Float16 h0 = f16_no_subnormal(v0), h1 = f16_no_subnormal(v1);
        const float d0 = v0 - (float)h0, d1 = v1 - (float)h1;
        const float s2 = wave_sum_canonical(__builtin_fmaf(v0, v0, v1 * v1));
        const float d2 = wave_sum_canonical(__builtin_fmaf(d0, d0, d1 * d1));
        const float m = wave_butterfly<OpMax>(fmaxf(fabsf(x.x), fabsf(x.y)));
        bad = __ballot(bad) != 0 || !(s2 - s2 == 0.f) || (s2 == 0.f && m > 0.f);
        const float rho = s2 > 0.f ? sqrtf(d2) * 1.001f / (sqrtf(s2) * 0.9999f) : 0.f;
        bad = bad || !(rho <= 9.765625e-4f);
        if (!bad) rho_w = fmaxf(rho_w, rho);
        const _Float16 nanh = (_Float16)__uint_as_float(0x7FC00000u);
        typedef _Float16 f16x2v __attribute__((ext_vector_type(2)));
        reinterpret_cast<f16x2v *>(Xh + (size_t)row * 128)[lane] = bad ? f16x2v{nanh, nanh} : f16x2v{h0, h1};
    }
    if (lane == 0 && rho_w > 0.f) atomicMax(rhoMax, __float_as_uint(rho_w));
}

hipError_t zh_launch_absmax(const float *dX, uint64_t n, uint32_t *dOut, hipStream_t s) {
    if (!n) return hipSuccess;
    hipLaunchKernelGGL(absmax_kernel, dim3((uint32_t)std::min<uint64_t>((n + 255) / 256, 256 * 16)), dim3(256), 0, s, dX, n, dOut);
    return hipGetLastError();
}
hipError_t zh_launch_row_half128(const float *dX, uint64_t row0, uint64_t n_rows, float sigma, void *dXh, uint32_t *dRhoMax, hipStream_t s) {
    if (!n_rows) return hipSuccess;
    hipLaunchKernelGGL(row_half128_kernel, dim3((uint32_t)std::min<uint64_t>((n_rows + 3) / 4, 256 * 32)), dim3(256), 0, s, dX, row0, n_rows, sigma,
                       (_Float16 *)dXh, dRhoMax);
    return hipGetLastError();
}

__global__ __launch_bounds__(256) void row_byte128_kernel(const float4 *__restrict__ X4, uint64_t n4, uint32_t *__restrict__ Xb,
                                                          uint32_t *__restrict__ notBytes) {
    bool bad = false;
    for (uint64_t i = (uint64_t)blockIdx.x * 256 + threadIdx.x; i < n4; i += (uint64_t)gridDim.x * 256) {
        const float4 v = X4[i];
        const float e[4] = {v.x, v.y, v.z, v.w};
        uint32_t w = 0;
#pragma unroll
        for (int j = 0; j < 4; j++) {
            const uint32_t b = (uint32_t)fminf(fmaxf(e[j], 0.f), 255.f);
            bad |= !((float)b == e[j]);
            w |= b << (8 * j);
        }
        Xb[i] = w;
    }
    if (__ballot(bad) != 0 && (threadIdx.x & 63) == 0) atomicOr(notBytes, 1u);
}
hipError_t zh_launch_row_byte128(const float *dX, uint64_t row0, uint64_t n_rows, void *dXb, uint32_t *dNotBytes, hipStream_t s) {
    if (!n_rows) return hipSuccess;
    const uint64_t n4 = n_rows * 32;
    hipLaunchKernelGGL(row_byte128_kernel, dim3((uint32_t)std::min<uint64_t>((n4 + 255) / 256, 256 * 32)), dim3(256), 0, s,
                       reinterpret_cast<const float4 *>(dX + (size_t)row0 * 128), n4, reinterpret_cast<uint32_t *>(dXb) + (size_t)row0 * 32, dNotBytes);
    return hipGetLastError();
}
__device__ __forceinline__ f16x8 bytes8_to_f16(uint32_t w0, uint32_t w1) {
    typedef _Float16 h2 __attribute__((ext_vector_type(2)));
    const h2 off = {(_Float16)-1024.f, (_Float16)-1024.f};
    const h2 a = __builtin_bit_cast(h2, __builtin_amdgcn_perm(0x64646464u, w0, 0x04010400u)) + off;
    const h2 b = __builtin_bit_cast(h2, __builtin_amdgcn_perm(0x64646464u, w0, 0x04030402u)) + off;
    const h2 c = __builtin_bit_cast(h2, __builtin_amdgcn_perm(0x64646464u, w1, 0x04010400u)) + off;
    const h2 d = __builtin_bit_cast(h2, __builtin_amdgcn_perm(0x64646464u, w1, 0x04030402u)) + off;
// ... 1046 lines not shown
                    list[off[j]] = pack(rl, eB0[j], slot);
                }
                for (uint32_t sidx = 1; sidx < c; sidx++) {
                    const ZhGroup *gp = groups + gb + sidx / GRP;
                    const uint64_t slot = gp->key_off[sidx % GRP] + eWithin[j];
                    list[off[j] + sidx] = pack(rl, gp->b[sidx % GRP], slot);
                }
            }
        }
        __builtin_amdgcn_fence(__ATOMIC_RELEASE, "wavefront");
        __builtin_amdgcn_wave_barrier();
        auto r_row = [](uint64_t r) { return (uint32_t)(r >> 60); };
        auto r_b = [](uint64_t r) { return (uint32_t)(r >> 36) & 0xFFFFFFu; };
        uint64_t rec = list[g < P ? g : P - 1];
        Ops cur;
        fetch(r_row(rec), r_b(rec), cur);
        for (uint32_t p = 0; p < P; p += G) {
            const uint32_t pn = p + G + g;
            const uint64_t recn = list[pn < P ? pn : P - 1];
            Ops nxt;
            fetch(r_row(recn), r_b(recn), nxt);
            const float s = dot8(cur);
            stash(s, r_row(rec), r_b(rec), rec & 0xFFFFFFFFFull, p + g < P);
            rec = recn; cur = nxt;
        }
    } else {
#pragma unroll
        for (int j = 0; j < ZH_SCAN_NE; j++) {
            unsigned long long m = __ballot(eC[j] != 0);
            while (m) {
                const int ll = __builtin_ctzll(m);
                m &= m - 1;
                const uint32_t c = (uint32_t)__builtin_amdgcn_readlane((int)eC[j], ll);
                const uint32_t gb = (uint32_t)__builtin_amdgcn_readlane((int)eGb[j], ll);
                const uint32_t w = (uint32_t)__builtin_amdgcn_readlane((int)eWithin[j], ll);
                const uint32_t rl = ((uint32_t)ll + 64u * j) / T;
                for (uint32_t s0 = 0; s0 < c; s0 += G) {
                    const uint32_t sidx = s0 + g < c ? s0 + g : c - 1;
                    const ZhGroup *gp = groups + gb + sidx / GRP;
                    const uint32_t b = gp->b[sidx % GRP];
                    Ops o;
                    fetch(rl, b, o);
                    const float s = dot8(o);
                    stash(s, rl, b, gp->key_off[sidx % GRP] + w, s0 + g < c);
                }
            }
        }
    }
    flush();
}

template <int D, int G>
static hipError_t launch_scan_approx_d(const float *dX, uint64_t n_rows, const ZhApprox &ap, const uint2 *dRowLeaf, uint32_t T,
                                       const uint32_t *dVisitBits, const uint4 *dNodeVisit, const ZhGroup *dGroups, uint32_t group,
                                       int metric, int mode, hipStream_t s) {
    const uint32_t RW = zh_scan_rows_per_wave(T);
    uint64_t rows_per_launch = zh_sweep_rows_per_launch(D);
    rows_per_launch = rows_per_launch / (4 * RW) * (4 * RW);
    const float Kc = zh_approx_bound(metric, D, 0);
    const int kinda = metric == ZH_COSINE ? (mode == ZH_COSINE_PARITY ? 2 : 1) : 0;
    for (uint64_t r = 0; r < n_rows; r += rows_per_launch) {
        const uint64_t r_end = r + rows_per_launch < n_rows ? r + rows_per_launch : n_rows;
        const uint64_t waves = (r_end - r + RW - 1) / RW, blocks = (waves + 3) / 4;
        if (blocks > 0x7FFFFFFFull) return hipErrorInvalidValue;
#define ZH_APX_LAUNCH(KA) \
        hipLaunchKernelGGL((scan_approx_kernel<D, G, KA>), dim3((uint32_t)blocks), dim3(256), 0, s, dX, (const uint4 *)ap.Qh, ap.qmeta, dRowLeaf, T, \
                           RW, dVisitBits, dNodeVisit, dGroups, group, r, r_end, Kc, ap.iv)
        if (kinda == 0) ZH_APX_LAUNCH(0);
        else if (kinda == 1) ZH_APX_LAUNCH(1);
        else ZH_APX_LAUNCH(2);
#undef ZH_APX_LAUNCH
    }
    return hipGetLastError();
}

bool zh_scan_mfma_supported(uint32_t d, uint32_t T) { return (d == 256 || d == 384 || d == 512 || d == 768 || d == 1024) && zh_scan_rows_per_wave(T) == 16; }
bool zh_scan_approx_supported(uint32_t d, uint32_t T, int metric) {
    if (metric != ZH_L2 && metric != ZH_L2SQ && metric != ZH_COSINE) return false;
    return zh_approx_groups(d) != 0 && zh_scan_rows_per_wave(T) != 0;
}

hipError_t zh_launch_scan_approx(const float *dX, uint32_t d, uint64_t n_rows, ZhApprox ap, const uint2 *dRowLeaf, uint32_t T,
                                 const uint32_t *dVisitBits, const uint4 *dNodeVisit, const ZhGroup *dGroups, uint32_t group, int metric,
                                 int mode, hipStream_t s) {
    if (!n_rows) return hipSuccess;
    if (ap.mfma) switch (d) {
    case 256: return launch_scan_mfma_d<256>(dX, n_rows, ap, dRowLeaf, T, dVisitBits, dNodeVisit, dGroups, group, s);
    case 384: return launch_scan_mfma_d<384>(dX, n_rows, ap, dRowLeaf, T, dVisitBits, dNodeVisit, dGroups, group, s);
    case 512: return launch_scan_mfma_d<512>(dX, n_rows, ap, dRowLeaf, T, dVisitBits, dNodeVisit, dGroups, group, s);
    case 768: return launch_scan_mfma_d<768>(dX, n_rows, ap, dRowLeaf, T, dVisitBits, dNodeVisit, dGroups, group, s);
    case 1024: return launch_scan_mfma_d<1024>(dX, n_rows, ap, dRowLeaf, T, dVisitBits, dNodeVisit, dGroups, group, s);
    default: return hipErrorInvalidValue;
    }
    switch (d) {
    case 128: {
        const uint32_t RW = zh_scan_rows_per_wave(T);
        uint64_t rows_per_launch = zh_sweep_rows_per_launch(128);
        rows_per_launch = rows_per_launch / (4 * RW) * (4 * RW);
        const float Kc = zh_approx_bound(metric, 128, 0);
        const int kinda = metric == ZH_COSINE ? (mode == ZH_COSINE_PARITY ? 2 : 1) : 0;
        for (uint64_t r = 0; r < n_rows; r += rows_per_launch) {
            const uint64_t r_end = r + rows_per_launch < n_rows ? r + rows_per_launch : n_rows;
            const uint64_t waves = (r_end - r + RW - 1) / RW, blocks = (waves + 3) / 4;
            if (blocks > 0x7FFFFFFFull) return hipErrorInvalidValue;
#define ZH_APX_LAUNCH(KA) \
            hipLaunchKernelGGL((scan_approx128_kernel<ZH_APX_G128, KA>), dim3((uint32_t)blocks), dim3(256), 0, s, dX, (const uint4 *)ap.Qh, ap.qmeta, dRowLeaf, T, RW, \
                               dVisitBits, dNodeVisit, dGroups, group, r, r_end, Kc, ap.iv)
            if (kinda == 0) ZH_APX_LAUNCH(0);
            else if (kinda == 1) ZH_APX_LAUNCH(1);
            else ZH_APX_LAUNCH(2);
#undef ZH_APX_LAUNCH
        }
        return hipGetLastError();
    }
    case 256: return launch_scan_approx_d<256, 4>(dX, n_rows, ap, dRowLeaf, T, dVisitBits, dNodeVisit, dGroups, group, metric, mode, s);
    case 384: return launch_scan_approx_d<384, 4>(dX, n_rows, ap, dRowLeaf, T, dVisitBits, dNodeVisit, dGroups, group, metric, mode, s);
    case 512: return launch_scan_approx_d<512, 2>(dX, n_rows, ap, dRowLeaf, T, dVisitBits, dNodeVisit, dGroups, group, metric, mode, s);
    case 768: return launch_scan_approx_d<768, ZH_APX_G768>(dX, n_rows, ap, dRowLeaf, T, dVisitBits, dNodeVisit, dGroups, group, metric, mode, s);
    case 1024: return launch_scan_approx_d<1024, 2>(dX, n_rows, ap, dRowLeaf, T, dVisitBits, dNodeVisit, dGroups, group, metric, mode, s);
    default: return hipErrorInvalidValue;
    }
}

#define ZH_APX_RADIX_SELECT(n, need_in, VAL, result)                                                        \
    {                                                                                                       \
        uint32_t prefix_ = 0, need_ = (need_in);                                                            \
        for (int sh_ = 24; sh_ >= 0; sh_ -= 8) {                                                            \
            __syncthreads();                                                                                \
            hist[tid] = 0;                                                                                  \
            __syncthreads();                                                                                \
            const uint32_t himask_ = sh_ == 24 ? 0u : (0xFFFFFFFFu << (sh_ + 8));                           \
            for (uint32_t i_ = tid; i_ < (n); i_ += 256) {                                                  \
                const uint32_t x_ = (VAL(i_));                                                              \
                if ((x_ & himask_) == prefix_) atomicAdd(&hist[(x_ >> sh_) & 255u], 1u);                    \
            }                                                                                               \
            __syncthreads();                                                                                \
            if (tid < 64) {                            \
                const uint32_t h0_ = hist[4 * tid], h1_ = hist[4 * tid + 1], h2_ = hist[4 * tid + 2], h3_ = hist[4 * tid + 3]; \
                const uint32_t ss_ = h0_ + h1_ + h2_ + h3_;                                                 \
                uint32_t inc_ = ss_;                                                                        \
                for (int m_ = 1; m_ < 64; m_ <<= 1) {                                                       \
                    const uint32_t t_ = __shfl_up(inc_, m_);                                                \
                    if ((int)tid >= m_) inc_ += t_;                                                         \
                }                                                                                           \
                const uint32_t exc_ = inc_ - ss_;                                                           \
                if (exc_ < need_ && need_ <= inc_) {                                                        \
                    uint32_t c_ = exc_, j_ = 4 * tid;                                                       \
                    if (need_ > c_ + h0_) { c_ += h0_; j_++;                                                \
                        if (need_ > c_ + h1_) { c_ += h1_; j_++;                                            \
                            if (need_ > c_ + h2_) { c_ += h2_; j_++; } } }                                  \
                    s_u[6] = j_; s_u[7] = c_;                                                               \
                }                                                                                           \
            }                                                                                               \
            __syncthreads();                                                                                \
            prefix_ |= s_u[6] << sh_;                                                                       \
            need_ -= s_u[7];                                                                                \
        }                                                                                                   \
        (result) = prefix_;                                                                                 \
    }

template <int KINDA>
__global__ __launch_bounds__(256) void select_tau_kernel(const ZhVisit *__restrict__ visits, uint64_t n_visits, uint32_t chunk,
                                                          uint32_t k_top, float Kc, ZhApprox ap) {
    __shared__ uint32_t hist[256];
    __shared__ uint32_t s_u[8];
    const uint32_t tid = threadIdx.x;
    const uint64_t base = (uint64_t)blockIdx.x * chunk;
    const uint32_t cnt = (uint32_t)(n_visits - base < chunk ? n_visits - base : chunk);
    for (uint32_t c = 0; c < cnt; c++) {
        const ZhVisit v = visits[base + c];
        if (v.take) {
            const float4 qm = ap.qmeta[v.b];
            uint64_t *__restrict__ raw = ap.iv + v.row_off;
            for (uint32_t i = tid; i < v.len; i += 256) {
                const uint64_t w = raw[i];
                raw[i] = approx_interval<KINDA>(__uint_as_float((uint32_t)w), __uint_as_float((uint32_t)(w >> 32)), qm, Kc, ap.row_rho, ap.rho_norm);
            }
            __syncthreads();
        }
        uint32_t tau = 0xFFFFFFFFu;
        if (v.take && v.take < v.len) {
            if (v.take < k_top) {
                if (tid == 0) {
                    const uint32_t slot = atomicAdd(&ap.ctl[0], 1u);
                    const uint32_t eb = atomicAdd(&ap.ctl[2], v.len);
                    if (slot >= ap.ex_cap) atomicOr(&ap.ctl[1], 4u);
                    else if ((uint64_t)eb + v.len > ap.ex_rows_cap) { atomicOr(&ap.ctl[1], 8u); ap.ex_visits[slot] = make_uint2(0xFFFFFFFFu, 0u); }
                    else ap.ex_visits[slot] = make_uint2((uint32_t)(base + c), eb);
                    ap.tauv[base + c] = 0u;
                }
                continue;
            }
            const uint64_t *__restrict__ kp = ap.iv + v.row_off;
#define ZH_APX_HI(i) ((uint32_t)(kp[i] >> 32))
            ZH_APX_RADIX_SELECT(v.len, v.take, ZH_APX_HI, tau);
#undef ZH_APX_HI
            if (tid == 0) atomicMin(&ap.qtau[v.b], tau);
        }
        if (tid == 0) ap.tauv[base + c] = tau;
    }
}

__global__ __launch_bounds__(256) void select_emit_kernel(const ZhVisit *__restrict__ visits, uint64_t n_visits, uint32_t chunk,
                                                           uint32_t k_top, const uint32_t *__restrict__ leaf_ids, ZhApprox ap) {
    __shared__ uint32_t s_u[8];
    const uint32_t tid = threadIdx.x;
    const uint64_t base = (uint64_t)blockIdx.x * chunk;
    const uint32_t cnt = (uint32_t)(n_visits - base < chunk ? n_visits - base : chunk);
    for (uint32_t c = 0; c < cnt; c++) {
        const ZhVisit v = visits[base + c];
        if (!v.take || (v.take < v.len && v.take < k_top)) continue;
        const uint64_t *__restrict__ kp = ap.iv + v.row_off;
        const uint32_t tv = ap.tauv[base + c], tq = ap.qtau[v.b];
        const uint32_t tau = tv < tq ? tv : tq;
        __syncthreads();
        if (tid == 0) { s_u[0] = 0; s_u[2] = 0; }
        __syncthreads();
        uint32_t mine = 0;
        for (uint32_t i = tid; i < v.len; i += 256) mine += ((uint32_t)kp[i] <= tau) ? 1u : 0u;
        if (mine) atomicAdd(&s_u[0], mine);
        __syncthreads();
        const uint32_t M = s_u[0];
        if (!M) continue;
        if (tid == 0) {
            const uint32_t b0 = atomicAdd(&ap.qcount[v.b], M);
            s_u[1] = b0;
            if (b0 + M > ap.capq) atomicOr(&ap.ctl[1], 1u);
        }
        __syncthreads();
        const uint32_t b0 = s_u[1];
        if (b0 + M <= ap.capq) {
            const size_t ob = (size_t)v.b * ap.capq + b0;
            for (uint32_t i = tid; i < v.len; i += 256) {
                const uint64_t w = kp[i];
                if ((uint32_t)w <= tau) {
                    const uint32_t pos = atomicAdd(&s_u[2], 1u);
                    ap.list_lo[ob + pos] = (uint32_t)w;
                    ap.list_hi[ob + pos] = (uint32_t)(w >> 32);
                    ap.list_id[ob + pos] = leaf_ids[(size_t)v.leaf_off + i];
                }
            }
        }
    }
}

template <int KIND>
__global__ __launch_bounds__(256) void exact_keys_kernel(const ZhVisit *__restrict__ visits, const float *__restrict__ X, uint32_t d,
                                                          const float *__restrict__ Q, const float *__restrict__ QQ,
                                                          const uint32_t *__restrict__ leaf_ids, int metric, int param, ZhApprox ap) {
    const uint32_t lane = threadIdx.x & 63, wv = threadIdx.x >> 6;
    if (ap.ctl[0] > ap.ex_cap) return;
    const uint32_t total = ap.ctl[0];
    for (uint32_t e = blockIdx.x; e < total; e += gridDim.x) {
        const uint2 ev = ap.ex_visits[e];
        if (ev.x == 0xFFFFFFFFu) continue;
        const ZhVisit v = visits[ev.x];
        const uint32_t i0 = blockIdx.y * 256u + wv * 64u;
        for (uint32_t i = i0; i < v.len && i < i0 + 64u; i++) {
            const uint32_t id = leaf_ids[(size_t)v.leaf_off + i];
            float s0, s1;
            lane_sums_generic<KIND>(X + (size_t)id * d, Q + (size_t)v.b * d, d, lane, param, s0, s1);
            if (lane == 0) ap.ex_keys[(size_t)ev.y + i] = key_of(metric, param, s0, s1, KIND == K_COS ? QQ[v.b] : 0.f);
        }
    }
}

__global__ __launch_bounds__(256) void exact_visit_kernel(const ZhVisit *__restrict__ visits, const uint32_t *__restrict__ leaf_ids, ZhApprox ap) {
    __shared__ uint64_t sk[2048];
    __shared__ __attribute__((aligned(16))) uint32_t si[2048];
    __shared__ uint32_t s_u32[8];
    __shared__ uint64_t s_red[8];
    const uint32_t tid = threadIdx.x, lane = tid & 63, wv = tid >> 6;
    if (ap.ctl[0] > ap.ex_cap) return;
    const uint32_t total = ap.ctl[0];
    for (uint32_t e = blockIdx.x; e < total; e += gridDim.x) {
        const uint2 ev = ap.ex_visits[e];
        if (ev.x == 0xFFFFFFFFu) continue;
        const ZhVisit v = visits[ev.x];
        const uint32_t eb = ev.y;
        __syncthreads();
        ZhVisit v2 = v;
        v2.row_off = eb; v2.cand_off = eb;
        bool need_slow = false;
        select_fast<false>(v2, leaf_ids, ap.ex_keys, ap.ex_ckeys, ap.ex_cids, sk, si, s_u32, need_slow);
        if (need_slow) {
            __syncthreads();
            select_slow(v2, leaf_ids, ap.ex_keys, ap.ex_ckeys, ap.ex_cids, sk, si, 2048);
        }
        __syncthreads();
        uint64_t tk = 0, ti = 0;
        for (uint32_t i = tid; i < v.take; i += 256) {
            const uint64_t kk = ap.ex_ckeys[(size_t)eb + i], ii = ap.ex_cids[(size_t)eb + i];
            if (kk > tk || (kk == tk && ii > ti)) { tk = kk; ti = ii; }
        }
        for (int m = 1; m < 64; m <<= 1) {
            const uint64_t ok = __shfl_xor(tk, m), oi = __shfl_xor(ti, m);
            if (ok > tk || (ok == tk && oi > ti)) { tk = ok; ti = oi; }
        }
        if (lane == 0) { s_red[wv] = tk; s_red[4 + wv] = ti; }
        __syncthreads();
        tk = s_red[0]; ti = s_red[4];
        for (int w = 1; w < 4; w++)
            if (s_red[w] > tk || (s_red[w] == tk && s_red[4 + w] > ti)) { tk = s_red[w]; ti = s_red[4 + w]; }
        if (tid == 0) s_u32[7] = 0;
        __syncthreads();
        const uint32_t tq = ap.qtau[v.b];
        uint32_t mine = 0;
        for (uint32_t i = tid; i < v.len; i += 256) {
            const uint64_t kk = ap.ex_keys[(size_t)eb + i];
            const uint32_t id = leaf_ids[(size_t)v.leaf_off + i];
            if ((kk < tk || (kk == tk && id <= ti)) && (uint32_t)ap.iv[v.row_off + i] <= tq) mine++;
        }
        if (mine) atomicAdd(&s_u32[7], mine);
        __syncthreads();
        const uint32_t M = s_u32[7];
        __syncthreads();
        if (tid == 0) {
            const uint32_t b0 = M ? atomicAdd(&ap.qcount[v.b], M) : 0u;
            s_u32[6] = b0; s_u32[7] = 0;
            if (M && b0 + M > ap.capq) atomicOr(&ap.ctl[1], 1u);
        }
        __syncthreads();
        const uint32_t b0 = s_u32[6];
        if (M && b0 + M <= ap.capq) {
            const size_t ob = (size_t)v.b * ap.capq + b0;
            for (uint32_t i = tid; i < v.len; i += 256) {
                const uint64_t kk = ap.ex_keys[(size_t)eb + i];
                const uint32_t id = leaf_ids[(size_t)v.leaf_off + i];
                const uint64_t w = ap.iv[v.row_off + i];
                if ((kk < tk || (kk == tk && id <= ti)) && (uint32_t)w <= tq) {
                    const uint32_t pos = atomicAdd(&s_u32[7], 1u);
                    ap.list_lo[ob + pos] = (uint32_t)w;
                    ap.list_hi[ob + pos] = (uint32_t)(w >> 32);
                    ap.list_id[ob + pos] = id;
                }
            }
        }
        __syncthreads();
    }
}

template <int D, int KIND>
__device__ __forceinline__ uint64_t exact_key(const float *__restrict__ X, uint32_t d, uint32_t id, const float *__restrict__ q,
                                              const float4 *qreg, float qq, uint32_t lane, int metric, int param) {
    float s0 = 0.f, s1 = 0.f;
    if constexpr (D > 0) {
        constexpr int NV = RowVec<D>::NV;
        float4 v[NV];
        load_row<D>(X + (size_t)id * D, lane, v);
        row_pair_sums<D, KIND>(v, qreg, lane, param, s0, s1);
        if (KIND == K_COS) {
            float4 c = make_float4(0.f, 0.f, 0.f, 0.f);
#pragma unroll
            for (int j = 0; j < NV; j++) {
                const bool act = (j < RowVec<D>::NJ) || (lane < (uint32_t)RowVec<D>::REM4);
                if (act) sq4(v[j], c);
            }
            s1 = wave_sum_canonical((c.x + c.y) + (c.z + c.w));
        }
    } else
        lane_sums_generic<KIND>(X + (size_t)id * d, q, d, lane, param, s0, s1);
    return key_of(metric, param, s0, s1, qq);
}

template <int LCAP>
__global__ __launch_bounds__(256) void final_survivors_kernel(uint32_t B, uint32_t k, ZhApprox ap, uint32_t only) {
    __shared__ uint64_t sk[LCAP];
    __shared__ uint32_t sl[LCAP];
    __shared__ uint32_t hist[256], scan[256], s_u[8];
    const uint32_t b = blockIdx.x, tid = threadIdx.x;
    if (ap.ctl[1] & (1u | 4u | 8u)) return;
    uint32_t n = ap.qcount[b];
    if (n > ap.capq) n = ap.capq;
    if ((only == 1 && n > 4096u) || (only == 2 && n <= 4096u)) return;
    if (n > (uint32_t)LCAP) n = LCAP;
    const size_t ob = (size_t)b * ap.capq;
    for (uint32_t i = tid; i < n; i += 256) {
        sk[i] = ((uint64_t)ap.list_id[ob + i] << 32) | ap.list_hi[ob + i];
        sl[i] = ap.list_lo[ob + i];
    }
    const uint32_t np2 = next_pow2(n);
    for (uint32_t i = n + tid; i < np2; i += 256) { sk[i] = ~0ull; sl[i] = ~0u; }
    block_bitonic_sort<uint32_t>(sk, sl, np2);
    constexpr uint32_t PER = LCAP / 256;
    uint64_t ek[PER];
    uint32_t el[PER], cntl = 0;
    bool keep[PER];
#pragma unroll
    for (uint32_t j = 0; j < PER; j++) {
        const uint32_t i = tid * PER + j;
        keep[j] = i < n && (i == 0 || (uint32_t)(sk[i] >> 32) != (uint32_t)(sk[i - 1] >> 32));
        ek[j] = i < n ? sk[i] : 0ull;
        el[j] = i < n ? sl[i] : 0u;
        cntl += keep[j] ? 1u : 0u;
    }
    auto block_scan = [&](uint32_t mine) {
        scan[tid] = mine;
        __syncthreads();
        for (uint32_t o = 1; o < 256; o <<= 1) {
            const uint32_t a = tid >= o ? scan[tid - o] : 0;
            __syncthreads();
            scan[tid] += a;
            __syncthreads();
        }
        return scan[tid] - mine;
    };
    uint32_t rank = block_scan(cntl);
    const uint32_t nu = scan[255];
    __syncthreads();
#pragma unroll
    for (uint32_t j = 0; j < PER; j++)
        if (keep[j]) { sk[rank] = ek[j]; sl[rank] = el[j]; rank++; }
    __syncthreads();
// ... 135 lines not shown
```

### zebra_amd/csrc/zh_internal.h

```cpp
#pragma once
#include <hip/hip_runtime.h>
#include <stddef.h>
#include <stdint.h>

#include "../../include/zebra_hip.h"

int zh_set_error(int code, const char *fmt, ...) __attribute__((format(printf, 2, 3)));
double zh_index_visits_per_pair(zh_index *ix);
void zh_search_ctx_abandon(zh_search_ctx *c);
void zh_search_ctx_stream_ordered(zh_search_ctx *c);

struct ZhVisit {
    uint32_t b;
    uint32_t leaf_off;
    uint32_t len;
    uint32_t take;
    uint64_t row_off;
    uint64_t cand_off;
    uint32_t node;
    uint32_t pad;
};

#define ZH_GROUP_MAX 4
struct ZhGroup {
// ... 108 lines not shown
                               hipStream_t s);
hipError_t zh_launch_walk_emit(ZhForestDev f, const float *dQ, uint32_t B, uint32_t d, int32_t n,
                               const uint32_t *dBits, uint32_t words_per_q, uint32_t P_dense,
                               const ZhPairCounts *dCounts, const ZhVisit *dInline, const uint64_t *dRowBase,
                               const uint64_t *dCandBase, const uint64_t *dVisitBase, ZhVisit *dVisits,
                               const uint32_t *dLeafCount, uint32_t *dLeafFill, const uint32_t *dGroupBase,
                               const uint64_t *dGroupRowBase, ZhGroup *dGroups, uint64_t *dGroupRowOff, hipStream_t s);
hipError_t zh_launch_sweep(const float *dX, uint32_t d, const float *dQ, const float *dQQ, const ZhGroup *dGroups,
                           const uint64_t *dGroupRowOff, uint64_t n_groups, const uint32_t *dWaveGroup,
                           const uint32_t *dLeafIds, uint64_t R_grouped, int metric, int mode, uint64_t *dKeys,
                           hipStream_t s, const uint32_t *dRunIf = nullptr);
bool zh_sweep_has_predicate(uint32_t d, int metric);
hipError_t zh_launch_wave_groups(const ZhGroup *dGroups, const uint64_t *dGroupRowOff, uint64_t n_groups, uint32_t *dWaveGroup,
                                 hipStream_t s);
#define ZH_SCAN_NE 4
bool zh_scan_sweep_supported(uint32_t d, uint32_t T, int metric);
uint32_t zh_scan_rows_per_wave(uint32_t T);
hipError_t zh_launch_row_leaf(const int4 *dNodePack, const uint32_t *dNodeTree, uint32_t n_nodes, const uint32_t *dLeafIds,
                              uint32_t T, uint64_t n_rows, uint2 *dRowLeaf, hipStream_t s);
hipError_t zh_launch_node_visits(const uint32_t *dLeafCount, const uint32_t *dGroupBase, const ZhGroup *dGroups, uint32_t n_nodes,
                                 uint32_t *dBits, uint4 *dNodeVisit, hipStream_t s);
hipError_t zh_launch_scan_sweep(const float *dX, uint32_t d, uint64_t n_rows, const float *dQ, const float *dQQ,
                                const uint2 *dRowLeaf, uint32_t T, const uint32_t *dVisitBits, const uint4 *dNodeVisit,
                                const ZhGroup *dGroups, uint32_t group, int metric, int param, uint64_t *dKeys,
                                const uint32_t *dRunIf , hipStream_t s);
uint64_t zh_sweep_rows_per_launch(uint32_t d);
hipError_t zh_launch_select(const ZhVisit *dVisits, uint64_t n_visits, const uint32_t *dLeafIds,
                            const uint64_t *dKeys, uint64_t *dCandKeys, uint32_t *dCandIds, uint32_t max_leaf_len,
                            const uint32_t *dRunIf, hipStream_t s);
hipError_t zh_launch_final(const uint64_t *dCandBase, uint32_t B, uint32_t T, uint32_t k, const uint64_t *dCandKeys,
                           const uint32_t *dCandIds, uint64_t id_base, uint64_t *dOutIds, uint64_t *dOutKeys,
                           uint32_t *dOutCounts, const uint32_t *dRunIf, hipStream_t s);
hipError_t zh_launch_merge(uint32_t S, uint32_t B, uint32_t k, const uint64_t *dIds, const uint64_t *dKeys,
                           const uint32_t *dCounts, uint64_t *dOutIds, uint64_t *dOutKeys, uint32_t *dOutCounts,
                           uint64_t stride64, uint64_t stride32, hipStream_t s);
#define ZH_DISTANCE_SCRATCH_BYTES (sizeof(ZhGroup) + 16)
hipError_t zh_launch_distance_rows(const float *dX, uint64_t n, uint32_t d, const float *dq, int metric, int mode,
                                   uint64_t *dKeys, void *dScratch, hipStream_t s);

#define ZH_APX_CTL_WORDS 8
struct ZhApprox {
    const void *Qh;
    const float4 *qmeta;
    uint64_t *iv;
    uint32_t *list_lo, *list_hi, *list_id;
    uint32_t *qcount;
    uint32_t capq;
    uint32_t *tauv;
    uint32_t *qtau;
    uint2 *ex_visits;
    uint32_t ex_cap;
    uint64_t *ex_keys, *ex_ckeys;
    uint32_t *ex_cids;
    uint32_t ex_rows_cap;
    uint32_t *ctl;
    const void *row_half;
    const float2 *row_meta;
    float row_rho;
    float rho_norm;
    uint32_t mfma;
    uint32_t n_queries;
    uint64_t iv_cap;
    float nx_max;
};
uint32_t zh_approx_groups(uint32_t d);
bool zh_approx_pays(uint32_t d);
float zh_approx_bound(int metric, uint32_t d, int mfma);
bool zh_scan_mfma_supported(uint32_t d, uint32_t T);
hipError_t zh_launch_row_half(const float *dX, uint64_t row0, uint64_t n_rows, uint32_t d, void *dXh, float2 *dRowMeta, uint32_t *dRhoMax,
                              const uint32_t *dPerm , uint64_t perm_rows, hipStream_t s);
hipError_t zh_launch_scan_order(const uint2 *dRowLeaf, uint64_t n_rows, uint32_t T, uint32_t n_keys, uint32_t *dPerm, hipStream_t s);
hipError_t zh_launch_order_agreement(const uint2 *dRowLeaf, const uint32_t *dPerm, uint64_t n_rows, uint32_t T, unsigned long long *dOut, hipStream_t s);
hipError_t zh_launch_permute_row_leaf(const uint2 *dRowLeaf, const uint32_t *dPerm, uint64_t perm_rows, uint64_t n_rows, uint32_t T, uint2 *dOut, hipStream_t s);
bool zh_scan_approx_supported(uint32_t d, uint32_t T, int metric);
hipError_t zh_launch_qhalf(const float *dQ, uint32_t B, uint32_t d, void *dQh, float4 *dQmeta, int layout, hipStream_t s);
hipError_t zh_launch_absmax(const float *dX, uint64_t n, uint32_t *dOut, hipStream_t s);
hipError_t zh_launch_row_half128(const float *dX, uint64_t row0, uint64_t n_rows, float sigma, void *dXh, uint32_t *dRhoMax, hipStream_t s);
hipError_t zh_launch_sweep128h(const void *dXh, const void *dQh, float inv, const ZhGroup *dGroups, const uint64_t *dGroupRowOff, uint64_t n_groups,
                               const uint32_t *dWaveGroup, const uint32_t *dLeafIds, uint64_t R_grouped, uint64_t *dIv, hipStream_t s,
                               const ZhApprox *fuse = nullptr, int fuse_kinda = 0, uint32_t k_top = 0, float Kc = 0.f, bool byte_rows = false);
uint64_t zh_sweep128h_rows_per_launch(bool lean, bool byte_rows);
hipError_t zh_launch_row_byte128(const float *dX, uint64_t row0, uint64_t n_rows, void *dXb, uint32_t *dNotBytes, hipStream_t s);
hipError_t zh_launch_exact_register(const ZhVisit *dVisits, uint64_t n_visits, uint32_t k, ZhApprox ap, hipStream_t s);
hipError_t zh_launch_scan_approx(const float *dX, uint32_t d, uint64_t n_rows, ZhApprox ap, const uint2 *dRowLeaf, uint32_t T,
                                 const uint32_t *dVisitBits, const uint4 *dNodeVisit, const ZhGroup *dGroups, uint32_t group, int metric,
                                 int mode, hipStream_t s);
hipError_t zh_launch_select_interval(const ZhVisit *dVisits, uint64_t n_visits, uint32_t k, const uint32_t *dLeafIds, ZhApprox ap,
                                     int metric, int mode, uint32_t d, hipStream_t s);
hipError_t zh_launch_final_interval(const ZhVisit *dVisits, const float *dX, uint32_t d, const float *dQ, const float *dQQ, uint32_t B,
                                    uint32_t k, const uint32_t *dLeafIds, int metric, int mode, uint64_t id_base, ZhApprox ap,
                                    uint64_t *dOutIds, uint64_t *dOutKeys, uint32_t *dOutCounts, uint32_t max_leaf_len, hipStream_t s);

hipError_t zh_launch_exact_score(const float *dX, uint32_t d, const uint32_t *dLive, uint64_t p0, uint32_t nr, const float *dQ,
                                 const float *dQQ, uint32_t B, int metric, int param, uint64_t *dKeys, uint64_t ld, hipStream_t s);
hipError_t zh_launch_exact_visits(uint32_t B, uint32_t nsub, uint32_t nr, uint32_t L, uint32_t k, uint64_t p0, uint64_t ld, ZhVisit *dVisits,
                                  uint64_t *dCandBase, hipStream_t s);
struct ZhExact2 {
    const void *Xh; const float2 *rowMeta; const uint32_t *perm; uint64_t perm_rows; const uint32_t *liveBits;
    const void *Qh; const float4 *qmeta; uint32_t B; float Kc, rho;
    uint32_t *tau, *cnt, *lid, *llo, *lhi; uint32_t cap; uint32_t *over;
};
bool zh_exact_mfma_supported(uint32_t d, int metric);
hipError_t zh_launch_exact_mfma(uint32_t d, int metric, int mode, const ZhExact2 &e, uint64_t p_begin, uint64_t p_end, hipStream_t s);
hipError_t zh_launch_exact_prune(const ZhExact2 &e, uint32_t k, uint32_t *dScratch, hipStream_t s);
hipError_t zh_launch_exact_survivor_keys(const float *dX, uint32_t d, const float *dQ, const float *dQQ, int metric, int mode, const ZhExact2 &e,
                                         uint64_t *dCKeys, uint32_t *dCIds, hipStream_t s);
hipError_t zh_launch_exact_empty(uint32_t B, uint32_t k, uint64_t *dIds, uint64_t *dKeys, uint32_t *dCounts, hipStream_t s);

struct ZhPrefilter {
    const float *S;
    uint32_t Bp;
    const float4 *leaf_meta;
    const float *qnorm;
    uint32_t *rows, *counts;
    float *tau;
    uint32_t cap;
    uint4 *amb;
    uint32_t amb_cap;
    uint32_t *ctl;
};
float zh_prefilter_bound(int metric, uint32_t d);
hipError_t zh_launch_leaf_meta(const uint32_t *dLeafIds, uint64_t n, const float *dHalfN2, const float *dNorm, float4 *dOut, hipStream_t s);
hipError_t zh_launch_prefilter(ZhForestDev f, uint32_t d, uint32_t B, uint32_t k, int metric, int mode, const ZhPairCounts *dCounts,
                               const ZhVisit *dInline, ZhWalkLog log, ZhPrefilter pf, hipStream_t s);
hipError_t zh_launch_prefilter_exact(ZhForestDev f, uint32_t d, const float *dX, const float *dQ, const float *dQQ, uint32_t B, int metric,
                                     int mode, uint64_t id_base, ZhPrefilter pf, uint64_t *dKeys, uint64_t *dIds, hipStream_t s);
hipError_t zh_launch_final_lists(uint32_t T, uint32_t B, uint32_t k, uint32_t cap, const uint64_t *dKeys, const uint64_t *dIds,
                                 const uint32_t *dCounts, uint64_t *dOutIds, uint64_t *dOutKeys, uint32_t *dOutCounts,
                                 uint32_t *dOver , hipStream_t s);
hipError_t zh_launch_row_norms(const float *dX, uint64_t n, uint32_t d, float *dHalfN2 , float *dNorm, hipStream_t s);
hipError_t zh_launch_row_scores4(const float *dX, uint64_t n, uint32_t d, const float *dQ4, float *dS, hipStream_t s);
hipError_t zh_launch_plane_hab(const uint2 *dSamples, uint32_t P, const float *dHalfN2, const float *dRowNorm, float4 *dOut, hipStream_t s);
hipError_t zh_launch_score_unc_fix(const float *dQ, uint32_t B, uint32_t d, const float *dPlanes, const float *dConsts, uint32_t P,
                                   uint32_t *dBits, const uint32_t *dUnc, uint32_t wpq, hipStream_t s);
hipError_t zh_launch_score_signs(const float *dS, uint32_t B, const uint2 *dSamples, uint32_t P, const float *dHalfN2, const float *dRowNorm,
                                 const float4 *dPlaneHab, const float *dQNorm, const float *dQ, uint32_t d, const float *dPlanes, const float *dConsts,
                                 uint32_t *dBits, uint32_t wpq, uint2 *dFixList, uint32_t fix_cap, unsigned long long *dFixCount, uint32_t *dUnc ,
                                 hipStream_t s);

struct ZhBuildNode {
    uint64_t seg_start;
    uint32_t len;
    uint32_t plane;
    uint64_t sample_a, sample_b;
    uint32_t first_chunk, n_chunks;
};
struct ZhBuildChunk {
    uint32_t node;
    uint32_t count;
    uint64_t pos;
};

struct ZhDescend {
    uint32_t row, node, depth, tree;
    uint64_t path;
};
hipError_t zh_launch_pack_nodes(const int32_t *dPlane, const int32_t *dLeft, const int32_t *dRight, const float *dConsts,
                                int4 *dPack, uint32_t n_nodes, hipStream_t s);
hipError_t zh_launch_descend(ZhForestDev f, const float *dX, uint32_t d, ZhDescend *dItems, uint32_t n, hipStream_t s);

hipError_t zh_launch_row_hash(const float *dX, uint64_t n, uint32_t d, uint64_t *dHash, hipStream_t s);

hipError_t zh_launch_rows_equal(const float *dX, uint32_t d, const uint32_t *dPairs, uint32_t n_pairs, uint8_t *dOut,
                                hipStream_t s);

hipError_t zh_launch_synth_rows(float *dX, uint64_t n, uint32_t d, uint64_t seed, uint64_t row0, int kind,
                                hipStream_t s);
hipError_t zh_launch_synth_queries(float *dOut, uint64_t seed_rows, uint64_t seed_q, uint64_t n_rows, uint64_t b0,
                                   uint64_t b, uint32_t d, int kind, hipStream_t s);
// ... 19 lines not shown
```

### zebra_amd/index.py

```python
import ctypes as C
from dataclasses import dataclass

import numpy as np

from . import _ffi
from ._ffi import check, lib


def _p(a):
    return a.ctypes.data_as(C.c_void_p)


def _f32(a, d=None):
    a = np.ascontiguousarray(a, dtype=np.float32)
    if d is not None and (a.ndim != 2 or a.shape[1] != d):
        raise ValueError(f"expected an (n, {d}) float32 array, got {a.shape}")
    return a


class _Metric:
    metric = None
    mode = _ffi.COSINE_PARITY

    def __init__(self, device=-1):
# ... 157 lines not shown
        check(lib().zh_index_deduplicate(self._h, _p(out), out.size, C.byref(n)))
        return out[:n.value]

    def compact(self):
        n = self.stored_rows()
        new_ids = np.empty(n, np.uint64)
        info = _ffi.CompactInfo()
        check(lib().zh_index_compact(self._h, _p(new_ids), n, C.byref(info)))
        return new_ids, info.as_dict()

    def set_forest(self, arrays):
        a = {k: np.ascontiguousarray(v) for k, v in arrays.items()}
        keep = [a["plane"].astype(np.int32), a["left"].astype(np.int32), a["right"].astype(np.int32),
                a["roots"].astype(np.uint32), _f32(a["planes"]).reshape(-1, self.dim), _f32(a["consts"]),
                a["leaf_ids"].astype(np.uint32)]
        fv = _ffi.ForestView(keep[0].size, keep[5].size, keep[3].size, keep[6].size, *[_p(x).value for x in keep])
        check(lib().zh_index_set_forest(self._h, C.byref(fv)))

    def get_forest(self):
        s = _ffi.ForestSizes()
        check(lib().zh_index_forest_sizes(self._h, C.byref(s)))
        out = dict(plane=np.empty(s.n_nodes, np.int32), left=np.empty(s.n_nodes, np.int32),
                   right=np.empty(s.n_nodes, np.int32), roots=np.empty(s.n_trees, np.uint32),
                   planes=np.empty((s.n_planes, self.dim), np.float32), consts=np.empty(s.n_planes, np.float32),
                   leaf_ids=np.empty(s.n_leaf_ids, np.uint32))
        check(lib().zh_index_get_forest(self._h, *[_p(out[k]) for k in
                                                  ("plane", "left", "right", "roots", "planes", "consts", "leaf_ids")]))
        return out

    def hash_signs(self, queries, dots=False):
        q = _f32(queries, self.dim)
        s = _ffi.ForestSizes()
        check(lib().zh_index_forest_sizes(self._h, C.byref(s)))
        words = (s.n_planes + 31) // 32
        bits = np.zeros((q.shape[0], max(words, 1)), np.uint32)
        dd = np.zeros((q.shape[0], s.n_planes), np.float32) if dots else None
        check(lib().zh_hash_signs(self._h, _p(q), q.shape[0], _p(bits), _p(dd) if dots else None))
        signs = np.unpackbits(bits.view(np.uint8), axis=1, bitorder="little")[:, :s.n_planes].astype(bool)
        return (signs, dd) if dots else signs

    def search_batch(self, queries, top_k, metric):
        q = _f32(queries, self.dim)
        b = q.shape[0]
        ids = np.empty((b, top_k), np.uint64)
        keys = np.empty((b, top_k), np.uint64)
        counts = np.zeros(b, np.uint32)
        check(lib().zh_search_batch(self._h, _p(q), b, top_k, metric.metric, metric.mode, _p(ids), _p(keys), _p(counts)))
        return ids, keys, counts

    def search(self, query, top_k, metric):
        ids, keys, counts = self.search_batch(_f32(query).reshape(1, -1), top_k, metric)
        n = int(counts[0])
        return list(zip(ids[0, :n].tolist(), keys[0, :n].tolist()))

    def search_batch_device(self, d_q_ptr, b, top_k, metric, d_ids_ptr, d_keys_ptr, d_counts_ptr, stream=None):
        check(lib().zh_search_batch_device(self._h, d_q_ptr, b, top_k, metric.metric, metric.mode, d_ids_ptr,
                                           d_keys_ptr, d_counts_ptr, stream))

    def search_exact_batch(self, queries, top_k, metric):
        q = _f32(queries, self.dim)
        b = q.shape[0]
        ids = np.empty((b, top_k), np.uint64)
        keys = np.empty((b, top_k), np.uint64)
        counts = np.zeros(b, np.uint32)
        check(lib().zh_search_exact_batch(self._h, _p(q), b, top_k, metric.metric, metric.mode, _p(ids), _p(keys), _p(counts)))
        return ids, keys, counts

    def search_exact(self, query, top_k, metric):
        ids, keys, counts = self.search_exact_batch(_f32(query).reshape(1, -1), top_k, metric)
        n = int(counts[0])
        return list(zip(ids[0, :n].tolist(), keys[0, :n].tolist()))

    def search_exact_batch_device(self, d_q_ptr, b, top_k, metric, d_ids_ptr, d_keys_ptr, d_counts_ptr, stream=None):
        check(lib().zh_search_exact_batch_device(self._h, d_q_ptr, b, top_k, metric.metric, metric.mode, d_ids_ptr,
                                                 d_keys_ptr, d_counts_ptr, stream))

    def exact_info(self):
        info = _ffi.ExactInfo()
        check(lib().zh_search_exact_info(self._h, C.byref(info)))
        return info.as_dict()

    def debug_keep_raw(self, on=True):
        check(lib().zh_debug_keep_raw(self._h, 1 if on else 0))

    def debug_scan_pairs(self, ctx=None):
        info = _ffi.DebugScanInfo()
        h = ctx._h if ctx is not None else None
        check(lib().zh_debug_scan_pairs(self._h, h, C.byref(info), None, 0, None))
        dt = np.dtype([("row", "<u4"), ("query", "<u4"), ("lo", "<u4"), ("hi", "<u4"), ("raw_s", "<f4"), ("raw_a2", "<f4"), ("flags", "<u4"), ("visit", "<u4")])
        assert dt.itemsize == C.sizeof(_ffi.DebugPair)
        pairs = np.zeros(int(info.pairs), dt)
        qmeta = np.zeros((int(info.queries), 4), np.float32)
        if info.approx_scan:
            check(lib().zh_debug_scan_pairs(self._h, h, C.byref(info), pairs.ctypes.data_as(C.c_void_p), pairs.shape[0], qmeta.ctypes.data_as(C.c_void_p)))
        return info.as_dict(), pairs, qmeta

    def read_rows(self, first, n):
        out = np.empty((n, self.dim), np.float32)
        check(lib().zh_index_read_rows(self._h, first, n, _p(out)))
        return out

    def search_context(self):
        return SearchContext(self)

    def sweep_stream(self):
        return lib().zh_index_sweep_stream(self._h)

    def rows_device_ptr(self):
        return lib().zh_index_rows_device(self._h)

    def set_profiling(self, level):
        check(lib().zh_set_profiling(self._h, level))

    def set_dense_levels(self, levels):
        check(lib().zh_set_dense_levels(self._h, levels))

    def set_sweep_mode(self, mode):
        check(lib().zh_set_sweep_mode(self._h, {"auto": 0, "leaf": 1, "scan": 2, "prefilter": 3, "approx": 4, "approx-valu": 5, "leaf-half": 6}.get(mode, mode)))

    def set_hash_mode(self, mode):
        check(lib().zh_set_hash_mode(self._h, {"auto": 0, "dense": 1, "scores": 2}.get(mode, mode)))

    def stats(self, reset=False):
        s = _ffi.Stats()
        check(lib().zh_stats(self._h, C.byref(s)))
        if reset:
            check(lib().zh_stats_reset(self._h))
        return s.as_dict()


class SearchContext:

    def __init__(self, index):
        self._index = index
        self._h = C.c_void_p()
        check(lib().zh_search_ctx_create(index._h, C.byref(self._h)))
        index._adopt(self)

    def begin(self, d_q_ptr, b, top_k, metric, stream=None):
        check(lib().zh_search_begin(self._h, d_q_ptr, b, top_k, metric.metric, metric.mode, stream))

    def finish(self, d_ids_ptr, d_keys_ptr, d_counts_ptr, sweep_stream=None):
        check(lib().zh_search_finish(self._h, d_ids_ptr, d_keys_ptr, d_counts_ptr, sweep_stream))

    def begin_window(self, d_q_ptrs, b, top_k, metric, stream=None):
        arr = (C.c_void_p * len(d_q_ptrs))(*d_q_ptrs)
        check(lib().zh_search_begin_window(self._h, arr, len(d_q_ptrs), b, top_k, metric.metric, metric.mode, stream))

    def finish_window(self, d_ids_ptrs, d_keys_ptrs, d_counts_ptrs, sweep_stream=None):
        n = len(d_ids_ptrs)
        a, b_, c = (C.c_void_p * n)(*d_ids_ptrs), (C.c_void_p * n)(*d_keys_ptrs), (C.c_void_p * n)(*d_counts_ptrs)
        check(lib().zh_search_finish_window(self._h, a, b_, c, sweep_stream))

    def wait(self):
        check(lib().zh_search_wait(self._h))

    def close(self):
        if getattr(self, "_h", None):
            lib().zh_search_ctx_destroy(self._h)
            self._h = None

    __del__ = close


UNIQUE_ID_BYTES = 128

# ... 146 lines not shown
```

Before: 201,800.

## Prune MFMA scan results using a per-query bound from the first launch

When the MFMA approximate scan is split across several launches, the first launch is made short. A new per-query kernel then computes a top-k threshold (tau) from its results using a shared-memory hash table and a radix select. Later launches skip storing scan words whose interval lower bound exceeds tau, and downstream select and register kernels treat unwritten (all-ones) slots as absent. This aims to cut candidate traffic and selection work. In exchange it adds a key-buffer memset, an extra kernel, per-store bound evaluation, and template variants.

```diff
diff --git a/include/zebra_hip.h b/include/zebra_hip.h
--- a/include/zebra_hip.h
+++ b/include/zebra_hip.h
@@ -275,6 +275,7 @@
     uint64_t pairs, visits;
 } zh_debug_scan_info;
 ZH_API int zh_debug_keep_raw(zh_index *idx, int on);
+ZH_API int zh_debug_scan_rows_per_launch(zh_index *idx, uint64_t rows);
 ZH_API int zh_debug_scan_pairs(zh_index *idx, zh_search_ctx *ctx, zh_debug_scan_info *info, zh_debug_pair *out, size_t cap, float *qmeta);
 
 ZH_API int zh_set_profiling(zh_index *idx, int level);
diff --git a/zebra_amd/_ffi.py b/zebra_amd/_ffi.py
--- a/zebra_amd/_ffi.py
+++ b/zebra_amd/_ffi.py
@@ -164,6 +164,7 @@
     ("zh_ref_header_decode", _i, [_vp, _sz, _i, _sz, _vp]),
     ("zh_ref_header_encode", _i, [_vp, _vp, _vp, _sz, _vp]),
     ("zh_debug_keep_raw", _i, [_vp, _i]),
+    ("zh_debug_scan_rows_per_launch", _i, [_vp, _u64]),
     ("zh_debug_scan_pairs", _i, [_vp, _vp, _vp, _vp, _sz, _vp]),
     ("zh_set_profiling", _i, [_vp, _i]),
     ("zh_stats", _i, [_vp, _vp]),
diff --git a/zebra_amd/csrc/zh_api.hip b/zebra_amd/csrc/zh_api.hip
--- a/zebra_amd/csrc/zh_api.hip
+++ b/zebra_amd/csrc/zh_api.hip
@@ -118,6 +118,7 @@
     bool scan = false;
     bool approx_f32rows = false;
     bool approx_fused = false;
+    bool scan_bound = false;
     bool approx_bytes = false;
     bool approx = false, approx_mfma = false, approx_leaf = false;
     uint32_t *h_ap = nullptr;
@@ -208,6 +209,7 @@
     bool rows_torn = false;
     int dense_levels = -1;
     bool debug_keep_raw = false;
+    uint64_t debug_scan_rows = 0;
     std::atomic<int> sweep_mode{0};
     std::atomic<uint32_t> approx_strikes{0};
     std::atomic<bool> mfma_f32_off{false};
@@ -2210,6 +2212,16 @@
         HIPCHK(hipMemsetAsync(c->wApCtl.p, 0, ZH_APX_CTL_WORDS * 4, s));
         HIPCHK(zh_launch_qhalf(c->dQ, (uint32_t)B, d, c->wQh.p, c->wQmeta.as<float4>(), c->approx_leaf ? 2 : (mfma ? 1 : 0), s));
     }
+    ZhScanBound sbound{};
+    sbound.rows_per_launch = ix->debug_scan_rows;
+    c->scan_bound = false;
+    if (c->approx && mfma && !c->approx_leaf) {
+        sbound.on = !ix->debug_keep_raw && tot.rows && zh_scan_mfma_launches(d, T, ix->n_rows, ix->debug_scan_rows) > 1;
+        sbound.visits = c->wVisits.as<ZhVisit>(); sbound.visitBase = c->wVisitBase.as<uint64_t>(); sbound.leaf_ids = f.leaf_ids;
+        sbound.T = T; sbound.k = (uint32_t)k;
+        if (sbound.on) HIPCHK(hipMemsetAsync(c->wKeys.p, 0xFF, tot.rows * 8, s));
+        c->scan_bound = sbound.on;
+    }
     HIPCHK(hipEventRecord(c->ev[2], s));
     hipStream_t hs = heavy ? heavy : s;
     if (hs != s) { HIPCHK(hipEventRecord(c->ev_emit, s)); HIPCHK(hipStreamWaitEvent(hs, c->ev_emit, 0)); }
@@ -2227,7 +2239,7 @@
                                    c->approx_fused ? &ap : nullptr, kinda, (uint32_t)k, zh_approx_bound(c->metric, d, 2), c->approx_bytes));
     else if (c->approx)
         HIPCHK(zh_launch_scan_approx(ix->X.as<float>(), d, ix->n_rows, ap, mfma ? scan_row_leaf : ix->row_leaf.as<uint2>(), T, c->wVisitBits.as<uint32_t>(),
-                                     c->wNodeVisit.as<uint4>(), c->wGroups.as<ZhGroup>(), f.group, c->metric, c->mode, hs));
+                                     c->wNodeVisit.as<uint4>(), c->wGroups.as<ZhGroup>(), f.group, c->metric, c->mode, hs, &sbound));
     else if (c->scan)
         HIPCHK(zh_launch_scan_sweep(ix->X.as<float>(), d, ix->n_rows, c->dQ, c->wQQ.as<float>(), ix->row_leaf.as<uint2>(), T,
                                     c->wVisitBits.as<uint32_t>(), c->wNodeVisit.as<uint4>(), c->wGroups.as<ZhGroup>(), f.group,
@@ -2504,6 +2516,12 @@
     ix->debug_keep_raw = on != 0;
     return ZH_OK;
 }
+extern "C" int zh_debug_scan_rows_per_launch(zh_index *ix, uint64_t rows) {
+    if (!ix) return fail(ZH_EINVAL, "zh_debug_scan_rows_per_launch: null index");
+    std::unique_lock<std::shared_mutex> lk(ix->mu);
+    ix->debug_scan_rows = rows;
+    return ZH_OK;
+}
 extern "C" int zh_debug_scan_pairs(zh_index *ix, zh_search_ctx *ctx, zh_debug_scan_info *info, zh_debug_pair *out, size_t cap, float *qmeta) {
     if (!ix || !info || (cap && !out)) return fail(ZH_EINVAL, "zh_debug_scan_pairs: null argument");
     std::unique_lock<std::shared_mutex> lk(ix->mu, std::defer_lock);
@@ -2546,6 +2564,7 @@
             o.row = lids[(size_t)z.leaf_off + i]; o.query = z.b; o.visit = (uint32_t)v; o.flags = fl;
             const uint64_t w = iv[z.row_off + i];
             o.lo = (uint32_t)w; o.hi = (uint32_t)(w >> 32);
+            if (c->scan_bound && w == ~0ull) o.flags |= 4u;
             o.raw_s = o.raw_a2 = 0.f;
             if (c->dbg_raw) { const uint64_t r = raw[z.row_off + i]; uint32_t a = (uint32_t)r, b2 = (uint32_t)(r >> 32); memcpy(&o.raw_s, &a, 4); memcpy(&o.raw_a2, &b2, 4); }
         }
diff --git a/zebra_amd/csrc/zh_approx.hip b/zebra_amd/csrc/zh_approx.hip
--- a/zebra_amd/csrc/zh_approx.hip
+++ b/zebra_amd/csrc/zh_approx.hip
@@ -1,4 +1,5 @@
 
+#include <algorithm>
 #include <cstdlib>
 
 #include "zh_internal.h"
@@ -437,7 +438,7 @@
 #ifndef ZH_MFMA_WAVES
 #define ZH_MFMA_WAVES 3
 #endif
-template <int D, bool F32ROWS>
+template <int D, bool F32ROWS, int BOUND>
 __global__ __launch_bounds__(256) __attribute__((amdgpu_waves_per_eu(D > 768 ? 2 : ZH_MFMA_WAVES, D > 768 ? 2 : ZH_MFMA_WAVES)))
 void scan_mfma_kernel(const u32x4v *__restrict__ Xh, const float *__restrict__ Xf, const float2 *__restrict__ rowMeta,
                                                          const uint4 *__restrict__ Qh, const uint2 *__restrict__ rowLeaf, uint32_t T,
@@ -445,7 +446,8 @@
                                                          const uint4 *__restrict__ nodeVisit, const ZhGroup *__restrict__ groups,
                                                          uint32_t GRP, uint64_t row_begin, uint64_t row_end, uint64_t *__restrict__ iv,
                                                          uint32_t *__restrict__ colStats ,
-                                                         uint32_t nq, uint64_t iv_cap, uint32_t *__restrict__ guard) {
+                                                         uint32_t nq, uint64_t iv_cap, uint32_t *__restrict__ guard,
+                                                         const uint32_t *__restrict__ qtau, const float4 *__restrict__ qmeta, float Kc, float rho) {
     constexpr int NS = D / 32;
     constexpr int NL = D / 64;
     constexpr int CL = ZH_MFMA_CL ? ZH_MFMA_CL : (NL % 4 == 0 ? 2 : 3);
@@ -463,6 +465,22 @@
     const uint64_t r0 = row_begin + wave * RW;
     if (r0 >= row_end) return;
     SP(const uint64_t sp0 = clock64();)
+    auto result_word = [](float sv, const float2 rm) {
+        const uint64_t w = ((uint64_t)__float_as_uint(rm.x) << 32) | __float_as_uint(sv * rm.y);
+        return w == ~0ull ? 0xFFFFFFFF7FC00000ull : w;
+    };
+    auto ruled_out = [&](uint64_t w, const float4 qm, uint32_t tau) {
+        if constexpr (BOUND >= 0) {
+#if defined(ZH_BOUND_EXP) && ZH_BOUND_EXP == 1
+            return tau != 0xFFFFFFFFu;
+#elif defined(ZH_BOUND_EXP) && ZH_BOUND_EXP == 2
+            return (uint32_t)approx_interval<(BOUND >= 0 ? BOUND : 0)>(__uint_as_float((uint32_t)w), __uint_as_float((uint32_t)(w >> 32)), qm, Kc, rho, 0.f) > tau && tau == 0x12345u;
+#endif
+            return (uint32_t)approx_interval<(BOUND >= 0 ? BOUND : 0)>(__uint_as_float((uint32_t)w), __uint_as_float((uint32_t)(w >> 32)), qm, Kc, rho, 0.f) > tau;
+        }
+        else
+            return false;
+    };
     const uint32_t nr = (uint32_t)(row_end - r0 < RW ? row_end - r0 : RW);
     const uint32_t n_ent = nr * T;
     const uint2 *__restrict__ ent = rowLeaf + (size_t)r0 * T;
@@ -568,14 +586,15 @@
             acc[st & 3] = __builtin_amdgcn_mfma_f32_16x16x32_f16(A[st], __builtin_bit_cast(f16x8, v), acc[st & 3], 0, 0, 0);
         }
     };
-    auto emit = [&](const f32x4v *acc, uint32_t rl, uint64_t slot, bool valid) {
+    auto emit = [&](const f32x4v *acc, uint32_t rl, uint64_t slot, bool valid, uint32_t b) {
         const f32x4v t = (acc[0] + acc[1]) + (acc[2] + acc[3]);
         if (valid && (rl >> 2) == h) {
             const uint32_t i = rl & 3u;
             const float sv = i == 0 ? t[0] : (i == 1 ? t[1] : (i == 2 ? t[2] : t[3]));
-            const float2 rm = rmeta[rl];
-            if (ZH_GUARD(slot < iv_cap, 2u))
-                __builtin_nontemporal_store(((uint64_t)__float_as_uint(rm.x) << 32) | __float_as_uint(sv * rm.y), iv + slot);
+            const uint64_t w = result_word(sv, rmeta[rl]);
+            bool out = false;
+            if constexpr (BOUND >= 0) out = ruled_out(w, qmeta[b], qtau[b]);
+            if (!out && ZH_GUARD(slot < iv_cap, 2u)) __builtin_nontemporal_store(w, iv + slot);
         }
     };
     if (listed) {
@@ -667,6 +686,11 @@
         f32x4v *al = acc_lds[wid];
         for (uint32_t t = 0; t < nt; t++) {
             f32x4v acc[4] = {{0.f, 0.f, 0.f, 0.f}, {0.f, 0.f, 0.f, 0.f}, {0.f, 0.f, 0.f, 0.f}, {0.f, 0.f, 0.f, 0.f}};
+            float4 cqm = make_float4(0.f, 0.f, 0.f, 0.f);
+            uint32_t ctau = 0xFFFFFFFFu;
+            if constexpr (BOUND >= 0) {
+                if (lane < 16) { const uint32_t cb = col_b(t, lane); cqm = qmeta[cb]; ctau = qtau[cb]; }
+            }
 #pragma unroll
             for (int c = 0; c < NCH; c += 2) {
                 issue(bA, bB, c + 1, rb);
@@ -684,13 +708,19 @@
             __builtin_amdgcn_fence(__ATOMIC_RELEASE, "wavefront");
             __builtin_amdgcn_wave_barrier();
             const uint32_t pe = tstart[t + 1];
-            for (uint32_t pi = tstart[t] + lane; pi < pe; pi += 64) {
-                const uint64_t rec = tl[pi];
+            for (uint32_t p0 = tstart[t]; p0 < pe; p0 += 64) {
+                const uint32_t pi = p0 + lane;
+                const bool valid = pi < pe;
+                const uint64_t rec = valid ? tl[pi] : 0ull;
                 const uint32_t rl = (uint32_t)(rec >> 60), col = (uint32_t)(rec >> 36) & 15u;
                 const float sv = reinterpret_cast<const float *>(al)[col * 16 + rl];
-                const float2 rm = rmeta[rl];
-                if (ZH_GUARD((rec & 0xFFFFFFFFFull) < iv_cap, 2u))
-                    __builtin_nontemporal_store(((uint64_t)__float_as_uint(rm.x) << 32) | __float_as_uint(sv * rm.y), iv + (rec & 0xFFFFFFFFFull));
+                const uint64_t w = result_word(sv, rmeta[rl]);
+                bool out = false;
+                if constexpr (BOUND >= 0) {
+                    const float4 qm = make_float4(__shfl(cqm.x, (int)col), __shfl(cqm.y, (int)col), __shfl(cqm.z, (int)col), __shfl(cqm.w, (int)col));
+                    out = ruled_out(w, qm, (uint32_t)__shfl((int)ctau, (int)col));
+                }
+                if (valid && !out && ZH_GUARD((rec & 0xFFFFFFFFFull) < iv_cap, 2u)) __builtin_nontemporal_store(w, iv + (rec & 0xFFFFFFFFFull));
             }
             __builtin_amdgcn_wave_barrier();
         }
@@ -727,29 +757,78 @@
                         mfma_chunk(cc, acc);
                         __builtin_amdgcn_sched_barrier(0);
                     }
-                    emit(acc, rl, gp->key_off[sidx % GRP] + w, s0 + c16 < c);
-                }
-            }
-        }
-    }
-}
+                    emit(acc, rl, gp->key_off[sidx % GRP] + w, s0 + c16 < c, gp->b[sidx % GRP]);
+                }
+            }
+        }
+    }
+}
+
+#ifndef ZH_SCAN_BOUND_FIRST16
+#define ZH_SCAN_BOUND_FIRST16 0
+#endif
+static uint32_t scan_launch_plan(uint64_t n_rows, uint64_t rpl, bool short_first, uint64_t *ends ) {
+    const uint64_t nl = (n_rows + rpl - 1) / rpl;
+    if (nl <= 1 || nl > 64 || !short_first) {
+        uint32_t n = 0;
+        for (uint64_t r = 0; r < n_rows && n < 64; r += rpl, n++) ends[n] = n < 63 && r + rpl < n_rows ? r + rpl : n_rows;
+        return n;
+    }
+    const uint64_t unit = rpl > 65536 ? 1024 : 64;
+    uint64_t first = (n_rows - (nl - 1) * rpl + 63) / 64 * 64, rest = rpl;
+    if (ZH_SCAN_BOUND_FIRST16) {
+        first = (n_rows / 16 + unit - 1) / unit * unit;
+        rest = ((n_rows - first) / (nl - 1) + unit - 1) / unit * unit;
+    }
+    uint32_t n = 0;
+    uint64_t r = first;
+    ends[n++] = r;
+    for (; r < n_rows && n < 64; n++) { r = n < 63 && r + rest < n_rows ? r + rest : n_rows; ends[n] = r; }
+    return n;
+}
+uint32_t zh_scan_mfma_launches(uint32_t d, uint32_t T, uint64_t n_rows, uint64_t rows_per_launch) {
+    const uint32_t RW = zh_scan_rows_per_wave(T);
+    if (!RW || !n_rows) return 0;
+    uint64_t rpl = rows_per_launch ? rows_per_launch : zh_sweep_rows_per_launch(d);
+    rpl = rpl / (4 * RW) * (4 * RW);
+    if (!rpl) rpl = 4 * RW;
+    return (uint32_t)std::min<uint64_t>((n_rows + rpl - 1) / rpl, 64);
+}
+
+static hipError_t launch_scan_bound(const ZhScanBound &sb, uint32_t B, const ZhApprox &ap, float Kc, int kinda, hipStream_t s);
 
 template <int D>
 static hipError_t launch_scan_mfma_d(const float *dX, uint64_t n_rows, const ZhApprox &ap, const uint2 *dRowLeaf, uint32_t T,
-                                     const uint32_t *dVisitBits, const uint4 *dNodeVisit, const ZhGroup *dGroups, uint32_t group, hipStream_t s) {
+                                     const uint32_t *dVisitBits, const uint4 *dNodeVisit, const ZhGroup *dGroups, uint32_t group, int metric, int mode,
+                                     const ZhScanBound &sb, hipStream_t s) {
     const uint32_t RW = zh_scan_rows_per_wave(T);
-    uint64_t rows_per_launch = zh_sweep_rows_per_launch(D);
+    uint64_t rows_per_launch = sb.rows_per_launch ? sb.rows_per_launch : zh_sweep_rows_per_launch(D);
     rows_per_launch = rows_per_launch / (4 * RW) * (4 * RW);
-    for (uint64_t r = 0; r < n_rows; r += rows_per_launch) {
-        const uint64_t r_end = r + rows_per_launch < n_rows ? r + rows_per_launch : n_rows;
+    if (!rows_per_launch) rows_per_launch = 4 * RW;
+    uint64_t ends[64];
+    const uint32_t nl = scan_launch_plan(n_rows, rows_per_launch, sb.on, ends);
+    const float Kc = zh_approx_bound(metric, D, 1);
+    const int kinda = metric == ZH_COSINE ? (mode == ZH_COSINE_PARITY ? 2 : 1) : 0;
+    uint64_t r = 0;
+    for (uint32_t li = 0; li < nl; li++) {
+        const uint64_t r_end = ends[li];
         const uint64_t waves = (r_end - r + RW - 1) / RW, blocks = (waves + 3) / 4;
         if (blocks > 0x7FFFFFFFull) return hipErrorInvalidValue;
-        if (ap.row_half)
-            hipLaunchKernelGGL((scan_mfma_kernel<D, false>), dim3((uint32_t)blocks), dim3(256), 0, s, (const u32x4v *)ap.row_half, dX, ap.row_meta, (const uint4 *)ap.Qh, dRowLeaf, T, RW,
-                               dVisitBits, dNodeVisit, dGroups, group, r, r_end, ap.iv, ap.ctl + 5, ap.n_queries, ap.iv_cap, ap.ctl + 7);
-        else
-            hipLaunchKernelGGL((scan_mfma_kernel<D, true>), dim3((uint32_t)blocks), dim3(256), 0, s, (const u32x4v *)nullptr, dX, ap.row_meta, (const uint4 *)ap.Qh, dRowLeaf, T, RW,
-                               dVisitBits, dNodeVisit, dGroups, group, r, r_end, ap.iv, ap.ctl + 5, ap.n_queries, ap.iv_cap, ap.ctl + 7);
+        const int bound = sb.on && li > 0 ? kinda : -1;
+#define ZH_MFMA_LAUNCH(F32, BD) \
+        hipLaunchKernelGGL((scan_mfma_kernel<D, F32, BD>), dim3((uint32_t)blocks), dim3(256), 0, s, (const u32x4v *)ap.row_half, dX, ap.row_meta, (const uint4 *)ap.Qh, dRowLeaf, \
+                           T, RW, dVisitBits, dNodeVisit, dGroups, group, r, r_end, ap.iv, ap.ctl + 5, ap.n_queries, ap.iv_cap, ap.ctl + 7, ap.qtau, ap.qmeta, Kc, ap.row_rho)
+        if (ap.row_half) {
+            if (bound < 0) ZH_MFMA_LAUNCH(false, -1); else if (bound == 0) ZH_MFMA_LAUNCH(false, 0); else if (bound == 1) ZH_MFMA_LAUNCH(false, 1); else ZH_MFMA_LAUNCH(false, 2);
+        } else {
+            if (bound < 0) ZH_MFMA_LAUNCH(true, -1); else if (bound == 0) ZH_MFMA_LAUNCH(true, 0); else if (bound == 1) ZH_MFMA_LAUNCH(true, 1); else ZH_MFMA_LAUNCH(true, 2);
+        }
+#undef ZH_MFMA_LAUNCH
+        if (sb.on && li == 0 && nl > 1) {
+            const hipError_t e = launch_scan_bound(sb, ap.n_queries, ap, Kc, kinda, s);
+            if (e != hipSuccess) return e;
+        }
+        r = r_end;
     }
     return hipGetLastError();
 }
@@ -1962,14 +2041,15 @@
 
 hipError_t zh_launch_scan_approx(const float *dX, uint32_t d, uint64_t n_rows, ZhApprox ap, const uint2 *dRowLeaf, uint32_t T,
                                  const uint32_t *dVisitBits, const uint4 *dNodeVisit, const ZhGroup *dGroups, uint32_t group, int metric,
-                                 int mode, hipStream_t s) {
+                                 int mode, hipStream_t s, const ZhScanBound *bound) {
     if (!n_rows) return hipSuccess;
+    const ZhScanBound sb = bound && ap.mfma ? *bound : ZhScanBound{};
     if (ap.mfma) switch (d) {
-    case 256: return launch_scan_mfma_d<256>(dX, n_rows, ap, dRowLeaf, T, dVisitBits, dNodeVisit, dGroups, group, s);
-    case 384: return launch_scan_mfma_d<384>(dX, n_rows, ap, dRowLeaf, T, dVisitBits, dNodeVisit, dGroups, group, s);
-    case 512: return launch_scan_mfma_d<512>(dX, n_rows, ap, dRowLeaf, T, dVisitBits, dNodeVisit, dGroups, group, s);
-    case 768: return launch_scan_mfma_d<768>(dX, n_rows, ap, dRowLeaf, T, dVisitBits, dNodeVisit, dGroups, group, s);
-    case 1024: return launch_scan_mfma_d<1024>(dX, n_rows, ap, dRowLeaf, T, dVisitBits, dNodeVisit, dGroups, group, s);
+    case 256: return launch_scan_mfma_d<256>(dX, n_rows, ap, dRowLeaf, T, dVisitBits, dNodeVisit, dGroups, group, metric, mode, sb, s);
+    case 384: return launch_scan_mfma_d<384>(dX, n_rows, ap, dRowLeaf, T, dVisitBits, dNodeVisit, dGroups, group, metric, mode, sb, s);
+    case 512: return launch_scan_mfma_d<512>(dX, n_rows, ap, dRowLeaf, T, dVisitBits, dNodeVisit, dGroups, group, metric, mode, sb, s);
+    case 768: return launch_scan_mfma_d<768>(dX, n_rows, ap, dRowLeaf, T, dVisitBits, dNodeVisit, dGroups, group, metric, mode, sb, s);
+    case 1024: return launch_scan_mfma_d<1024>(dX, n_rows, ap, dRowLeaf, T, dVisitBits, dNodeVisit, dGroups, group, metric, mode, sb, s);
     default: return hipErrorInvalidValue;
     }
     switch (d) {
@@ -2054,7 +2134,7 @@
             uint64_t *__restrict__ raw = ap.iv + v.row_off;
             for (uint32_t i = tid; i < v.len; i += 256) {
                 const uint64_t w = raw[i];
-                raw[i] = approx_interval<KINDA>(__uint_as_float((uint32_t)w), __uint_as_float((uint32_t)(w >> 32)), qm, Kc, ap.row_rho, ap.rho_norm);
+                if (w != ~0ull) raw[i] = approx_interval<KINDA>(__uint_as_float((uint32_t)w), __uint_as_float((uint32_t)(w >> 32)), qm, Kc, ap.row_rho, ap.rho_norm);
             }
             __syncthreads();
         }
@@ -2097,7 +2177,7 @@
         if (tid == 0) { s_u[0] = 0; s_u[2] = 0; }
         __syncthreads();
         uint32_t mine = 0;
-        for (uint32_t i = tid; i < v.len; i += 256) mine += ((uint32_t)kp[i] <= tau) ? 1u : 0u;
+        for (uint32_t i = tid; i < v.len; i += 256) { const uint64_t w = kp[i]; mine += ((uint32_t)w <= tau && w != ~0ull) ? 1u : 0u; }
         if (mine) atomicAdd(&s_u[0], mine);
         __syncthreads();
         const uint32_t M = s_u[0];
@@ -2113,7 +2193,7 @@
             const size_t ob = (size_t)v.b * ap.capq + b0;
             for (uint32_t i = tid; i < v.len; i += 256) {
                 const uint64_t w = kp[i];
-                if ((uint32_t)w <= tau) {
+                if ((uint32_t)w <= tau && w != ~0ull) {
                     const uint32_t pos = atomicAdd(&s_u[2], 1u);
                     ap.list_lo[ob + pos] = (uint32_t)w;
                     ap.list_hi[ob + pos] = (uint32_t)(w >> 32);
@@ -2122,6 +2202,80 @@
             }
         }
     }
+}
+
+#define ZH_SCAN_BOUND_SLOTS 8192u
+#define ZH_SCAN_BOUND_VISITS 512u
+template <int KINDA>
+__global__ __launch_bounds__(1024) void scan_bound_kernel(const ZhVisit *__restrict__ visits, const uint64_t *__restrict__ visitBase, uint32_t T, uint32_t k_top,
+                                                           const uint32_t *__restrict__ leaf_ids, float Kc, ZhApprox ap) {
+    __shared__ uint32_t t_id[ZH_SCAN_BOUND_SLOTS], t_hi[ZH_SCAN_BOUND_SLOTS];
+    __shared__ uint32_t v_off[ZH_SCAN_BOUND_VISITS + 1], v_leaf[ZH_SCAN_BOUND_VISITS];
+    __shared__ uint32_t hist[1024];
+    __shared__ uint32_t s_u[8];
+    const uint32_t tid = threadIdx.x, b = blockIdx.x;
+    const uint64_t v0 = visitBase[(uint64_t)b * T], v1 = visitBase[(uint64_t)(b + 1) * T];
+    const uint32_t nv = (uint32_t)(v1 - v0);
+    if (nv == 0 || nv > ZH_SCAN_BOUND_VISITS) return;
+    for (uint32_t i = tid; i < ZH_SCAN_BOUND_SLOTS; i += 1024) { t_id[i] = 0xFFFFFFFFu; t_hi[i] = 0xFFFFFFFFu; }
+    if (tid == 0) s_u[0] = 0;
+    const uint64_t base = visits[v0].row_off;
+    uint64_t run = 0;
+    for (uint32_t i = tid; i < nv; i += 1024) {
+        const ZhVisit v = visits[v0 + i];
+        v_off[i] = (uint32_t)(v.row_off - base);
+        v_leaf[i] = v.leaf_off | ((!v.take || (v.take < v.len && v.take < k_top)) ? 0x80000000u : 0u);
+        if (i == nv - 1) { run = v.row_off + v.len - base; v_off[nv] = (uint32_t)run; }
+    }
+    __syncthreads();
+    const uint32_t n = v_off[nv];
+    if (n >= 0x7FFFFFFFu) return;
+    const float4 qm = ap.qmeta[b];
+    const uint64_t *__restrict__ raw = ap.iv + base;
+    for (uint32_t s0 = 0; s0 < n; s0 += 8u * 1024u) {
+        uint64_t w[8];
+#pragma unroll
+        for (int j = 0; j < 8; j++) { const uint32_t si = s0 + 1024u * j + tid; w[j] = si < n ? raw[si] : ~0ull; }
+#pragma unroll
+        for (int j = 0; j < 8; j++) {
+            if (w[j] == ~0ull) continue;
+            const uint32_t si = s0 + 1024u * j + tid;
+            const uint32_t hi = (uint32_t)(approx_interval<KINDA>(__uint_as_float((uint32_t)w[j]), __uint_as_float((uint32_t)(w[j] >> 32)), qm, Kc, ap.row_rho, ap.rho_norm) >> 32);
+            if (hi == 0xFFFFFFFFu) continue;
+            uint32_t lo_v = 0, hi_v = nv;
+            while (hi_v - lo_v > 1) { const uint32_t mid = (lo_v + hi_v) >> 1; if (v_off[mid] <= si) lo_v = mid; else hi_v = mid; }
+            const uint32_t vl = v_leaf[lo_v];
+            if (vl & 0x80000000u) continue;
+            const uint32_t id = leaf_ids[(size_t)vl + (si - v_off[lo_v])];
+            uint32_t hs = (id * 2654435761u) >> 19;
+            for (uint32_t tries = 0; tries < ZH_SCAN_BOUND_SLOTS; tries++) {
+                uint32_t cur = *(volatile uint32_t *)&t_id[hs];
+                if (cur == 0xFFFFFFFFu) {
+                    if (*(volatile uint32_t *)&s_u[0] >= ZH_SCAN_BOUND_SLOTS * 3 / 4) break;
+                    cur = atomicCAS(&t_id[hs], 0xFFFFFFFFu, id);
+                    if (cur == 0xFFFFFFFFu) { atomicAdd(&s_u[0], 1u); cur = id; }
+                }
+                if (cur == id) { atomicMin(&t_hi[hs], hi); break; }
+                hs = (hs + 1u) & (ZH_SCAN_BOUND_SLOTS - 1u);
+            }
+        }
+    }
+    __syncthreads();
+    uint32_t tau = 0xFFFFFFFFu;
+    if (s_u[0] >= k_top) {
+        const uint32_t n_sel = tid < 256 ? ZH_SCAN_BOUND_SLOTS : 0u;
+#define ZH_APX_TV(i) (t_hi[i])
+        ZH_APX_RADIX_SELECT(n_sel, k_top, ZH_APX_TV, tau);
+#undef ZH_APX_TV
+    }
+    if (tid == 0 && tau != 0xFFFFFFFFu) atomicMin(&ap.qtau[b], tau);
+}
+static hipError_t launch_scan_bound(const ZhScanBound &sb, uint32_t B, const ZhApprox &ap, float Kc, int kinda, hipStream_t s) {
+    if (!B) return hipSuccess;
+    if (kinda == 0) hipLaunchKernelGGL(scan_bound_kernel<0>, dim3(B), dim3(1024), 0, s, sb.visits, sb.visitBase, sb.T, sb.k, sb.leaf_ids, Kc, ap);
+    else if (kinda == 1) hipLaunchKernelGGL(scan_bound_kernel<1>, dim3(B), dim3(1024), 0, s, sb.visits, sb.visitBase, sb.T, sb.k, sb.leaf_ids, Kc, ap);
+    else hipLaunchKernelGGL(scan_bound_kernel<2>, dim3(B), dim3(1024), 0, s, sb.visits, sb.visitBase, sb.T, sb.k, sb.leaf_ids, Kc, ap);
+    return hipGetLastError();
 }
 
 template <int KIND>
@@ -2189,7 +2343,8 @@
         for (uint32_t i = tid; i < v.len; i += 256) {
             const uint64_t kk = ap.ex_keys[(size_t)eb + i];
             const uint32_t id = leaf_ids[(size_t)v.leaf_off + i];
-            if ((kk < tk || (kk == tk && id <= ti)) && (uint32_t)ap.iv[v.row_off + i] <= tq) mine++;
+            const uint64_t w = ap.iv[v.row_off + i];
+            if ((kk < tk || (kk == tk && id <= ti)) && (uint32_t)w <= tq && w != ~0ull) mine++;
         }
         if (mine) atomicAdd(&s_u32[7], mine);
         __syncthreads();
@@ -2208,7 +2363,7 @@
                 const uint64_t kk = ap.ex_keys[(size_t)eb + i];
                 const uint32_t id = leaf_ids[(size_t)v.leaf_off + i];
                 const uint64_t w = ap.iv[v.row_off + i];
-                if ((kk < tk || (kk == tk && id <= ti)) && (uint32_t)w <= tq) {
+                if ((kk < tk || (kk == tk && id <= ti)) && (uint32_t)w <= tq && w != ~0ull) {
                     const uint32_t pos = atomicAdd(&s_u32[7], 1u);
                     ap.list_lo[ob + pos] = (uint32_t)w;
                     ap.list_hi[ob + pos] = (uint32_t)(w >> 32);
diff --git a/zebra_amd/csrc/zh_internal.h b/zebra_amd/csrc/zh_internal.h
--- a/zebra_amd/csrc/zh_internal.h
+++ b/zebra_amd/csrc/zh_internal.h
@@ -214,9 +214,18 @@
 uint64_t zh_sweep128h_rows_per_launch(bool lean, bool byte_rows);
 hipError_t zh_launch_row_byte128(const float *dX, uint64_t row0, uint64_t n_rows, void *dXb, uint32_t *dNotBytes, hipStream_t s);
 hipError_t zh_launch_exact_register(const ZhVisit *dVisits, uint64_t n_visits, uint32_t k, ZhApprox ap, hipStream_t s);
+struct ZhScanBound {
+    uint64_t rows_per_launch;
+    bool on;
+    const ZhVisit *visits;
+    const uint64_t *visitBase;
+    const uint32_t *leaf_ids;
+    uint32_t T, k;
+};
+uint32_t zh_scan_mfma_launches(uint32_t d, uint32_t T, uint64_t n_rows, uint64_t rows_per_launch);
 hipError_t zh_launch_scan_approx(const float *dX, uint32_t d, uint64_t n_rows, ZhApprox ap, const uint2 *dRowLeaf, uint32_t T,
                                  const uint32_t *dVisitBits, const uint4 *dNodeVisit, const ZhGroup *dGroups, uint32_t group, int metric,
-                                 int mode, hipStream_t s);
+                                 int mode, hipStream_t s, const ZhScanBound *bound = nullptr);
 hipError_t zh_launch_select_interval(const ZhVisit *dVisits, uint64_t n_visits, uint32_t k, const uint32_t *dLeafIds, ZhApprox ap,
                                      int metric, int mode, uint32_t d, hipStream_t s);
 hipError_t zh_launch_final_interval(const ZhVisit *dVisits, const float *dX, uint32_t d, const float *dQ, const float *dQQ, uint32_t B,
diff --git a/zebra_amd/index.py b/zebra_amd/index.py
--- a/zebra_amd/index.py
+++ b/zebra_amd/index.py
@@ -263,6 +263,9 @@
 
     def debug_keep_raw(self, on=True):
         check(lib().zh_debug_keep_raw(self._h, 1 if on else 0))
+
+    def debug_scan_rows_per_launch(self, rows=0):
+        check(lib().zh_debug_scan_rows_per_launch(self._h, int(rows)))
 
     def debug_scan_pairs(self, ctx=None):
         info = _ffi.DebugScanInfo()
```

New measurement: 160,100. 0.793x the previous value.
